# mir-group/allegro

Hardware: AMD Instinct MI355X
Metric: edge tensor-products/sec (forward+force) (higher is better)
Workload: dtype f32; 1 GPU; c4: bulk Si 23^3 cells (97 336 atoms), r_cut 5 A, l_max=2, L=2, u=64; atoms=97336, edges=2725408, parallelism=single GPU, weights=random init (reference initialisers), seed 456, workspace_bytes=21849491824

## Files before the change

### __graft_entry__.py

```python
import os
import sys

ROOT = os.path.dirname(os.path.abspath(__file__))
if ROOT not in sys.path:
    sys.path.insert(0, ROOT)


def build() -> None:
    from allegro_amd.build import build_library, build_torch_ops

    path = build_library(force=True)
    assert os.path.exists(path)
    assert os.path.exists(build_torch_ops(force=True))
    import ctypes

    lib = ctypes.CDLL(path)
    assert lib.aa_version() >= 1
    import allegro_amd
    import allegro_amd.nn
    from oracle import restatement

    print(f"[build] OK: {path}")


def smoke() -> None:
    import torch

    from oracle import restatement as R
    from tests.golden_utils import load_model_fixture
    from tests.hip_utils import fixture_data, model_from_fixture

    assert torch.cuda.is_available(), "smoke() needs a GPU"
    dev = torch.device("cuda:0")
    fx = load_model_fixture("c2", torch.float32)
    model = model_from_fixture(fx, torch.float32, device=dev)
    data, sv = fixture_data(fx, torch.float32, dev)
    g = model.prepare_graph(data["edge_index"], data["atom_types"], data["pos"].shape[0], sv)
    e_atom, forces = model.energy_forces(data["pos"], g)
    torch.cuda.synchronize()
    ref = R.allegro_energy_forces(fx["cfg"], fx["sd"], fx["pos"], fx["edge_index"], fx["types"], fx["shift_vec"])
    de = (e_atom.cpu() - ref["atomic_energy"].reshape(-1)).abs().max().item()
    df = (forces.cpu() - ref["forces"]).abs().max().item()
    dg = (forces.cpu() - fx["out"]["forces"]).abs().max().item()
    print(f"[smoke] C2 fp32 on {torch.cuda.get_device_name(0)}: max|dE_i|={de:.2e} max|dF| vs oracle={df:.2e} "
          f"vs reference golden={dg:.2e} eV/A")
    assert de < 1e-4 and df < 1e-4 and dg < 1e-4, "HIP path disagrees with the oracle"


if __name__ == "__main__":
    build()
    if "--smoke" in sys.argv:
        smoke()
```

### allegro_amd/_lib.py

```python
import ctypes as C
import os
from typing import Optional

import numpy as np

AA_MAX_LAYERS = 4
AA_MAX_MLP_LAYERS = 4
AA_F32, AA_F64 = 0, 1

_dp = C.POINTER(C.c_double)
_ip = C.POINTER(C.c_int32)


class TpDesc(C.Structure):
    _fields_ = [("mul", C.c_int32), ("d1", C.c_int32), ("d2", C.c_int32), ("dout", C.c_int32),
                ("num_paths", C.c_int32), ("coupling", C.c_int32), ("nnz", C.c_int32),
                ("nz_i", _ip), ("nz_j", _ip), ("nz_k", _ip), ("nz_path", _ip), ("nz_val", _dp)]


class ModelConfig(C.Structure):
    _fields_ = [("dtype", C.c_int32), ("num_types", C.c_int32), ("num_bessels", C.c_int32), ("poly_p", C.c_double),
                ("l_max", C.c_int32), ("num_layers", C.c_int32), ("num_scalar", C.c_int32), ("num_tensor", C.c_int32),
                ("embed_dim", C.c_int32), ("embed_mlp_depth", C.c_int32), ("embed_mlp_width", C.c_int32),
                ("latent_mlp_depth", C.c_int32), ("latent_mlp_width", C.c_int32),
                ("readout_mlp_depth", C.c_int32), ("readout_mlp_width", C.c_int32),
                ("forward_weight_init", C.c_int32), ("avg_num_neighbors", C.c_double), ("act_const", C.c_double),
                ("has_scales", C.c_int32), ("has_shifts", C.c_int32), ("tps", TpDesc * AA_MAX_LAYERS),
                ("embed_kind", C.c_int32), ("spline_span", C.c_int32), ("env_shared_weights", C.c_int32),
                ("act_kind", C.c_int32 * 3), ("act_consts", C.c_double * 3), ("bessel_convention", C.c_int32)]


class PlanOptions(C.Structure):
    _fields_ = [(n, C.c_int32) for n in (
        "tp_generic", "tp_no_chain", "tp_no_moments", "tp_no_operator", "tp_force_operator", "tp_operator_fused",
        "gemm_no_chain", "gemm_fp32_mfma", "gemm_valu", "gemm_v1", "gemm_lds_epilogue", "f64_column_loop",
        "embed_no_fuse", "fused_forward", "moments_waves_per_block", "f64_rows", "no_channel_padding", "poison_workspace", "no_slot_form", "op_proj_gemm", "op_env_vector", "staged_no_fold", "op_recompute_bvecs", "readout_two_pass", "tp_prefer_moments", "fused_narrow", "chain_staged_weights")]


def options_from_env() -> PlanOptions:
    env = os.environ
    flag = lambda k: int(env.get(k, "0")[:1] == "1")
    o = PlanOptions()
    o.tp_generic, o.tp_no_chain, o.tp_no_moments = flag("AA_TP_GENERIC"), flag("AA_TP_NOCHAIN"), flag("AA_TP_NOMOM")
    o.tp_no_operator, o.tp_force_operator, o.tp_operator_fused = flag("AA_TP_NOOP"), flag("AA_TP_OP"), flag("AA_OP_NOSPLIT")
    o.gemm_no_chain, o.gemm_fp32_mfma, o.gemm_valu, o.gemm_v1 = (flag("AA_GEMM_NOCHAIN"), flag("AA_GEMM_FP32_MFMA"),
                                                                 flag("AA_GEMM_VALU"), flag("AA_GEMM_V1"))
    o.gemm_lds_epilogue = int(env.get("AA_GEMM_DIRECT_EPILOGUE", "1")[:1] == "0")
    o.f64_column_loop = {"0": 1, "2": 2}.get(env.get("AA_F64_NLOOP", "1")[:1], 0)
    o.embed_no_fuse = flag("AA_EMBED_NOFUSE")
    o.fused_forward = {"0": 3, "1": 1, "2": 2, "4": 4}.get(env.get("AA_FUSED", "")[:1], 0)
    o.moments_waves_per_block = int(env.get("AA_MOM_WPB", "0") or 0)
    o.no_channel_padding = flag("AA_NO_PAD")
    o.no_slot_form = flag("AA_NO_SLOT_FORM")
    o.op_proj_gemm = {"1": 1, "0": 2}.get(env.get("AA_OP_PROJ", "")[:1], 0)
    o.op_env_vector = flag("AA_OP_ENV_VECTOR")
    o.staged_no_fold = flag("AA_STAGED_NOFOLD")
    o.op_recompute_bvecs = flag("AA_OP_RECOMPUTE_BVECS")
    o.readout_two_pass = flag("AA_READOUT_TWO_PASS")
    o.tp_prefer_moments = flag("AA_TP_PREFER_MOM")
    o.fused_narrow = {"1": 1, "2": 2, "3": 3, "4": 4}.get(env.get("AA_FUSED_NARROW", "")[:1], 0)
    o.chain_staged_weights = flag("AA_CHAIN_STAGED")
    o.poison_workspace = flag("AA_POISON")
    o.f64_rows = {"0": 2, "2": 1}.get(env.get("AA_F64_ROWS", "")[:1], 0)
    return o


class RawWeights(C.Structure):
    _fields_ = [("rmax_recip", _dp), ("bessel_weights", _dp), ("center_embed", _dp), ("neighbor_embed", _dp),
                ("basis_linear", _dp), ("embed_mlp", _dp * AA_MAX_MLP_LAYERS), ("env_embed_linear", _dp),
                ("first_proj", _dp), ("latent", (_dp * AA_MAX_MLP_LAYERS) * AA_MAX_LAYERS),
                ("tp_weights", _dp * AA_MAX_LAYERS), ("readout", _dp * AA_MAX_MLP_LAYERS), ("scales", _dp),
                ("shifts", _dp), ("spline_weights", _dp)]


class Graph(C.Structure):
    _fields_ = [("num_atoms", C.c_int64), ("num_edges", C.c_int64), ("center", C.c_void_p), ("nbr", C.c_void_p),
                ("rowptr", C.c_void_p), ("types", C.c_void_p), ("shift_vec", C.c_void_p),
                ("t_rowptr", C.c_void_p), ("t_perm", C.c_void_p), ("atom_begin", C.c_int64), ("atom_end", C.c_int64),
                ("max_degree", C.c_int64)]


class PairZbl(C.Structure):
    _fields_ = [("num_types", C.c_int32), ("atomic_numbers", _dp), ("qqr2e", C.c_double), ("poly_p", C.c_double)]


class GemmSeg(C.Structure):
    _fields_ = [("p", C.c_void_p), ("ld", C.c_int32), ("n", C.c_int32)]


class GemmDesc(C.Structure):
    _fields_ = [("dtype", C.c_int32), ("K", C.c_int32), ("N", C.c_int32), ("M", C.c_int64),
                ("a_count", C.c_int32), ("c_count", C.c_int32), ("a", GemmSeg * 3), ("c", GemmSeg * 3),
                ("c_accum", C.c_int32 * 3), ("has_z", C.c_int32), ("has_add", C.c_int32), ("z", GemmSeg * 3),
                ("add", GemmSeg * 3), ("act_a", C.c_int32), ("act_lo", C.c_int32), ("act_hi", C.c_int32),
                ("act_kind", C.c_int32), ("batch", C.c_int32), ("a_bs", C.c_int64), ("c_bs", C.c_int64),
                ("bsel4", C.c_uint64), ("num_weights", C.c_int32), ("weights", C.c_void_p), ("force_kernel", C.c_int32),
                ("v1", C.c_int32), ("lds_epilogue", C.c_int32), ("f64_rows", C.c_int32), ("f64_column_loop", C.c_int32)]


GEMM_FORMS = {name: i for i, name in enumerate((
    "NONE",
    "F64_VALU", "F64_MFMA", "F64_PIPE_GRID", "F64_PIPE_LOOP", "F64_ROWS_ACC", "F64_ROWS_OPND", "F64_ROWS_ACC_BATCHED",
    "F64_ROWS_OPND_BATCHED", "F64_VALU_EACH", "F64_MFMA_EACH", "F64_PIPE_GRID_EACH", "F64_PIPE_LOOP_EACH",
    "F32_VALU", "F32_MFMA_V1", "F32_V3_K2", "F32_V3_K4", "F32_V3_KS", "F32_BF16X3_K2", "F32_BF16X3_K4", "F32_BF16X3_KS",
    "F32_BF16X3_LDS_K2", "F32_BF16X3_LDS_K4", "F32_BF16X3_LDS_KS", "F32_BF16X3_BATCHED_K2", "F32_BF16X3_BATCHED_K4",
    "F32_BF16X3_BATCHED_KS", "F32_VALU_EACH", "F32_MFMA_V1_EACH", "F32_V3_EACH", "F32_BF16X3_LDS_EACH"))}


class AllegroError(RuntimeError):
    pass


def make_tp_desc(mul, d1, d2, dout, num_paths, coupling, nz_i, nz_j, nz_k, nz_path, nz_val):
    arrs = [np.ascontiguousarray(a, dtype=np.int32) for a in (nz_i, nz_j, nz_k, nz_path)]
    val = np.ascontiguousarray(nz_val, dtype=np.float64)
    d = TpDesc(int(mul), int(d1), int(d2), int(dout), int(num_paths), int(bool(coupling)), int(len(val)),
               arrs[0].ctypes.data_as(_ip), arrs[1].ctypes.data_as(_ip), arrs[2].ctypes.data_as(_ip),
               arrs[3].ctypes.data_as(_ip), val.ctypes.data_as(_dp))
    return d, arrs + [val]


class NlInput(C.Structure):
    _fields_ = [("num_atoms", C.c_int64), ("pos", C.c_void_p), ("cell", C.c_double * 9), ("pbc", C.c_int32 * 3),
                ("dtype", C.c_int32), ("r_cut", C.c_double)]


class NlTypes(C.Structure):
    _fields_ = [("num_types", C.c_int32), ("types_are_int64", C.c_int32), ("cutoffs", _dp), ("atom_types", C.c_void_p)]


class PruneInput(C.Structure):
    _fields_ = [("num_atoms", C.c_int64), ("num_edges", C.c_int64), ("pos", C.c_void_p), ("dtype", C.c_int32),
                ("rowptr", C.c_void_p), ("nbr", C.c_void_p), ("shift_vec", C.c_void_p)]


class EdgeList(C.Structure):
    _fields_ = [("num_atoms", C.c_int64), ("num_edges", C.c_int64), ("edge_index", C.c_void_p), ("row_stride", C.c_int64),
                ("index_is_int64", C.c_int32), ("dtype", C.c_int32), ("pos", C.c_void_p), ("shift_vec", C.c_void_p)]


class Frames(C.Structure):
    _fields_ = [("num_frames", C.c_int32), ("frame_atoms", C.c_void_p)]


# ... 233 lines not shown
```

### allegro_amd/csrc/aa_common.h

```cpp
#pragma once
#include <type_traits>
#include <hip/hip_runtime.h>

#include <algorithm>
#include <cmath>
#include <cstdint>
#include <cstdio>
#include <cstring>
#include <string>
#include <vector>

#include "allegro_amd.h"

extern __shared__ unsigned char aa_smem[];

namespace aa {

void set_error(const std::string& msg);
int fail(int code, const std::string& msg);
int device_cu_count();

#define AA_CHECK_HIP(expr)                                                                      \
  do {                                                                                          \
    hipError_t _e = (expr);                                                                     \
// ... 129 lines not shown
  sn = (q & 1) ? c : s;
  cs = (q & 1) ? s : c;
  if (q & 2) sn = -sn;
  if ((q + 1) & 2) cs = -cs;
}
__device__ __forceinline__ float aa_sin(float x) {
  float s, c;
  aa_sincos(x, s, c);
  return s;
}
__device__ __forceinline__ double aa_sin(double x) { return sin(x); }
__device__ __forceinline__ float aa_cos(float x) {
  float s, c;
  aa_sincos(x, s, c);
  return c;
}
__device__ __forceinline__ double aa_cos(double x) { return cos(x); }
__device__ __forceinline__ float aa_pow(float x, float y) {
  const int n = int(y);
  if (float(n) == y && n >= 0 && n <= 32) {
    float r = 1.f, b = x;
    for (int m = n; m; m >>= 1) {
      if (m & 1) r *= b;
      b *= b;
    }
    return r;
  }
  return powf(x, y);
}
__device__ __forceinline__ double aa_pow(double x, double y) { return pow(x, y); }
__device__ __forceinline__ float aa_sqrt(float x) { return sqrtf(x); }
__device__ __forceinline__ double aa_sqrt(double x) { return sqrt(x); }

__device__ __forceinline__ int sh_l_of(int i) { return i < 1 ? 0 : (i < 4 ? 1 : (i < 9 ? 2 : 3)); }

struct Seg {
  void* p;
  int ld;
  int n;
};
struct SegList {
  int count;
  Seg s[3];
};

struct GemmArgs {
  int64_t M;
  int K, N;
  SegList a;
  const void* B;
  const void* Bp;
  const void* Bq;
  SegList c;
  int c_accum[3];
  int has_z;
  SegList z;
  int act_a;
  int act_lo, act_hi;
  int has_add;
  SegList add;
  int force_kernel;
  int act_kind;
  int opt_v1, opt_lds_epilogue, opt_f64_column_loop, opt_f64_rows;
  int batch;
  int64_t a_bs, c_bs, b_bs, bp_bs, bq_bs;
  unsigned long long bsel4;
};
template <typename T>
int launch_gemm(const GemmArgs& g, hipStream_t stream);

struct ChainLayer {
  GemmArgs g;
  int use_prev;
  int keep_tile;
  int keep_act;
  int a_mode;
  const void* a2_add;
  const void* a2_z;
  int ld_a2add, ld_a2z;
  void* embrev_out;
  void* edge_sum_out;
  void* kept_out;
  int ld_kept;
};
struct ChainArgs {
  int64_t M;
  int nlayers;
  ChainLayer L[4];
  const void* ro_w;
  double ro_factor;
  const void* ro_scales;
  const int32_t* types;
  const int32_t* center;
  const int32_t* nbr;
  const void* emb_table;
  int num_types;
};
int launch_gemm_chain(const ChainArgs& c, hipStream_t stream);
struct ChainB2Args {
  int64_t M;
  const float* a;
  const float* add;
  const float* z;
  int lda, ldadd, ldz;
  const void* Wq;
  float* c0;
  float* c1;
  int ldc0, ldc1;
};
int launch_chain_b2_resident(const ChainB2Args& g, hipStream_t stream);
size_t gemm_packed_elems(int K, int N);
void gemm_pack_b(const double* B, int K, int N, double* out);
size_t gemm_bf16x3_words(int K, int N);
void gemm_pack_bf16x3(const float* B, int K, int N, unsigned* out);

struct TpGroup {
  int32_t out_idx;
  int32_t path;
  int32_t begin, end;
};
struct TpEntry {
  int32_t a, b;
  float val_f;
  double val_d;
};
struct TpTable {
  int32_t num_groups;
  const TpGroup* groups;
  const TpEntry* entries;
};
struct TpLayerDev {
  int32_t mul, d1, d2, dout, num_paths, coupling;
  TpTable fwd;
  TpTable bx1;
  TpTable bx2;
};

struct TpOperand {
  const void* dense;
  const void* sh;
  const void* w;
  int ldw;
  int ld_sh;
};
struct TpOperandGrad {
  void* dense;
  void* gw;
  int ldgw;
  void* gsh;
  int ld_gsh;
};

struct TpLayerFwdArgs {
  int64_t E, N;
  const int32_t* rowptr;
  const int32_t* eids;
  TpOperand x1, x2;
  const void* weights;
  double scatter_factor;
  void* x2s;
  void* out;
  void* scal;
  int ld_scal;
};
struct TpLayerBwdArgs {
  int64_t E, N;
// ... 55 lines not shown
  const void* weights;
  int coupling;
  double sf;
  void* x2s;
  void* out;
  void* scal;
  int ld_scal;
};
struct TpSpecBwdArgs {
  int64_t E, N;
  const int32_t* rowptr;
  int u;
  const void* sh;
  int ld_sh;
  const void* w_x1;
  int ld_w1;
  const void* x1_dense;
  const void* w_env;
  int ld_we;
  const void* weights;
  int coupling;
  double sf;
  const void* x2s;
  const void* gout;
  const void* gscal;
  int ld_gscal;
  void* g_x1_dense;
  void* g_w1;
  int ld_gw1;
  void* g_wenv;
  int ld_gwe;
  void* gsh_x1;
  void* gsh_env;
  int ld_gsh;
};
struct TpChainArgs {
  int64_t E, N;
  int64_t atom0;
  const int32_t* rowptr;
  int u;
  const void* sh;
  int ld_sh;
  const void* w0;
  int ld_w0;
  const void* wenv0;
  int ld_we0;
  const void* wenv1;
  int ld_we1;
  const void* weights0;
  const void* weights1;
  int coupling;
  double sf;
  const void* x2s0;
  void* x2s1;
  void* scal1;
  int ld_scal;
  const void* gscal0;
  const void* gscal1;
  int ld_gscal;
  void* g_w0;
  int ld_gw0;
  void* g_wenv;
  int ld_gwe;
  void* gsh_x1;
  void* gsh_env;
  int ld_gsh;
};
int find_chain_pair(int sig0, int sig1);

struct TpMomArgs {
  TpChainArgs c;
  const void* a0;
  int ld_a0, ka0;
  const void* a1;
  int ld_a1, ka1;
  const void* wk0;
  const void* wt0;
  const void* wk1;
  const void* wt1;
  void* g_a;
  int ld_ga;
  int ka_lds;
  int waves_per_block;
};
struct TpOpArgs {
  int64_t N, E;
  int64_t atom0;
  const int32_t* rowptr;
  int u;
  const void* sh;
  int ld_sh;
  const void* w0;
  int ld_w0;
  int coupling;
  double sf;
  const void* x2s[3];
  const void* tpw[3];
  const void* a;
  int ld_a, ka, act;
  const void* wk;
  const void* wt;
  void* scal;
  int ld_scal;
  const void* gscal[3];
  int ld_gscal;
  void* q;
  void* g_w0;
  int ld_gw0;
  void* gsh_x1;
  void* gsh_env;
  int ld_gsh;
  void* g_a;
  int ld_ga;
  int ka_lds;
  void* bvec;
  void* gmbuf;
  void* mbuf;
  int num_layers;
  int proj_gemm;
  void* dx2s;
  int env_mfma;
  int bvec_ready;
};
int find_op_chain(const int* sigs, int num_layers);
template <typename T>
int launch_tp_op(int chain, int layer, bool reverse, const TpOpArgs& a, hipStream_t stream, int phase = 0);

template <typename T>
int launch_tp_mom_fwd_first(int pair, const TpMomArgs& a, hipStream_t stream);
template <typename T>
int launch_tp_mom_fwd_last(int pair, const TpMomArgs& a, hipStream_t stream);
template <typename T>
int launch_tp_mom_bwd_last(int pair, const TpMomArgs& a, hipStream_t stream);
template <typename T>
int launch_tp_mom_bwd_first(int pair, const TpMomArgs& a, hipStream_t stream);
template <typename T>
int launch_tp_chain_fwd_last(int pair, const TpChainArgs& a, hipStream_t stream);
template <typename T>
int launch_tp_chain_bwd_last(int pair, const TpChainArgs& a, hipStream_t stream);
template <typename T>
int launch_tp_chain_bwd_first(int pair, const TpChainArgs& a, hipStream_t stream);

int find_spec_sig(const aa_tp_desc& d);

struct TpDenseArgs {
  int64_t E, N;
  const int32_t* rowptr;
  const int32_t* eids;
  int u, coupling;
  double sf;
  const void* x1;
  const void* x2;
  const void* weights;
  void* x2s;
  void* out;
  const void* gout;
  void* gx1;
  void* gx2;
};
bool tp_dense_supported(int sig, int u, int dtype);
template <typename T>
int launch_tp_dense(int sig, bool backward, const TpDenseArgs& a, hipStream_t stream);
template <typename T>
int launch_tp_dense_wgrad(int sig, int u, int coupling, const TpLayerWgradArgs& a, hipStream_t stream);
template <typename T>
int launch_tp_spec_fwd(int sig, const TpSpecFwdArgs& a, hipStream_t stream);
template <typename T>
int launch_tp_spec_bwd(int sig, const TpSpecBwdArgs& a, hipStream_t stream);

constexpr int kFusedMaxSteps = 56;
constexpr int kFusedKeepDefault = 2;
constexpr int kFusedMaxDegree = 128;
constexpr int kFusedTailAtomsPerCu = 64;
constexpr int kFusedTeamTilesSmall = 4096;
struct FusedFwdArgs {
  int64_t N, atom0, atom_end;
  int32_t* tile_atoms;
  int32_t* tile_counts;
  int64_t tile_cap;
  const int32_t *rowptr, *nbr, *types;
  const float* pos;
  const float* shift_vec;
  int num_types, embed_kind, spline_span;
  float poly_p;
  const float *rmax_recip, *bessel_w;
  const float* emb_tab;
  const void* wstep[kFusedMaxSteps][2];
  const float *tpw0, *tpw1;
  int coupling;
  float sf;
  const float* ro_w;
  float ro_factor;
  const float *scales, *shifts;
  float* vec;
  float* sh;
  float* se_h;
  float* emb;
  float* w0;
  float* lat_h0;
  float* lat_h1;
  float* ro_h;
  float* fcat;
  float *x2s0, *x2s1;
  float* atom_energy;
  int long_only;
  int32_t* status;
  int mixed;
  int skip_long, fill_done;
  float* g_fcat;
  float* g_scal1;
  int ld_gfcat;
  float* g_scal0;
  float* gsh_env1;
};
size_t fused_fwd_lds_bytes(int num_types, bool teams);
enum class FusedForm { OneWave, FourWave, EightWave, EightWaveTail, EightWaveDeepTail };
int fused_fwd_num_steps(int R);
int launch_fused_fwd(int pair, FusedForm form, const FusedFwdArgs& a, const FusedFwdArgs* wide, hipStream_t stream);
// ... 153 lines not shown
```

### allegro_amd/csrc/aa_gemm.hip

```cpp
#include "aa_common.h"
#include "aa_mfma.h"

namespace aa {


template <typename T>
__device__ __forceinline__ T seg_load(const SegList& sl, int64_t row, int col) {
  int c = col;
#pragma unroll
  for (int s = 0; s < 3; ++s) {
    if (s < sl.count) {
      if (c < sl.s[s].n) return static_cast<const T*>(sl.s[s].p)[row * sl.s[s].ld + c];
      c -= sl.s[s].n;
    }
  }
  return T(0);
}

__device__ __forceinline__ bool a_act(const GemmArgs& g, int k) { return g.act_a && (g.act_hi == 0 || (k >= g.act_lo && k < g.act_hi)); }

template <typename T>
__device__ __forceinline__ void seg_store(const GemmArgs& g, int64_t row, int col, T v) {
  int c = col;
#pragma unroll
// ... 939 lines not shown
#pragma unroll
        for (int q = 0; q < 6; ++q) {
          wn0[q] = p0[q * 64];
          wn1[q] = p1[q * 64];
        }
        __builtin_amdgcn_sched_barrier(0);
        v4f a2[4];
        const int k2 = kc + 2 < KC ? kc + 2 : KC - 1;
        load_a_frag_acc(g, gm, k2, hh, a2, a_sh);
        __builtin_amdgcn_sched_barrier(0);
        u32x4 x1[2], x2[2], x3[2];
        split3_pack(a0, x1, x2, x3);
        chunk_pair_bf16x3(wc0, wc1, x1, x2, x3, acc0, acc1);
#pragma unroll
        for (int q = 0; q < 4; ++q) {
          a0[q] = a1[q];
          a1[q] = a2[q];
        }
#pragma unroll
        for (int q = 0; q < 6; ++q) {
          wc0[q] = wn0[q];
          wc1[q] = wn1[q];
        }
      }
    }
    if (LDS_EPI) {
      store_pair_lds(g, acc0, acc1, two, reinterpret_cast<float*>(aa_smem) + wv * 32 * EP_LD, m0, nt * 32, lane);
    } else {
      store_tile_t(g, acc0, gm, nt * 32, lane, vec_ok, c_sh);
      if (two) store_tile_t(g, acc1, gm, nt * 32 + 32, lane, vec_ok, c_sh);
    }
  }
}


__device__ __forceinline__ void tile_epilogue_store(const GemmArgs& g, v16f& acc, int64_t gm, int n0, int lane) {
#pragma unroll
  for (int gq = 0; gq < 4; ++gq) {
    const int f0 = n0 + 8 * gq + 4 * (lane >> 5);
    const Dst4 d = resolve4(g, gm, f0);
    if (d.nvalid == 0) continue;
    v4f v = {acc[4 * gq], acc[4 * gq + 1], acc[4 * gq + 2], acc[4 * gq + 3]};
    if (d.add) {
      const v4f ad = *reinterpret_cast<const v4f*>(d.add);
#pragma unroll
      for (int e = 0; e < 4; ++e) v[e] += ad[e];
    }
    if (d.z) {
      const v4f z = *reinterpret_cast<const v4f*>(d.z);
#pragma unroll
      for (int e = 0; e < 4; ++e) v[e] *= dsilu(z[e]);
    }
#pragma unroll
    for (int e = 0; e < 4; ++e) acc[4 * gq + e] = v[e];
    if (d.c) {
      if (d.accum) {
        const v4f o = *reinterpret_cast<const v4f*>(d.c);
#pragma unroll
        for (int e = 0; e < 4; ++e) v[e] += o[e];
      }
      *reinterpret_cast<v4f*>(d.c) = v;
    }
  }
}

constexpr int kChainMaxBlocks = 12;
struct ChainTileDev {
  float* c;
  const float* z;
  const float* add;
  int ldc, ldz, ldadd, accum;
};
struct ChainLayerDev {
  const u32x4* Wq;
  int KCg, KC, NT;
  int keep_tile, keep_act, a_mode, pad_;
  int use_prev, pad2_;
  float* edge_sum_out;
  float* embrev_out;
  float* kept_out;
  int ld_kept, pad3_;
  const float *a2_add, *a2_z;
  int ld_a2add, ld_a2z;
  const float* a[kChainMaxBlocks];
  int lda[kChainMaxBlocks];
  ChainTileDev t[kChainMaxBlocks];
};
struct ChainDev {
  int64_t M;
  int nlayers;
  float ro_factor;
  const float* ro_w;
  const float* ro_scales;
  const int32_t* types;
  const int32_t* center;
  int ro_n;
  const int32_t* nbr;
  const float* emb_table;
  int num_types;
  ChainLayerDev L[4];
};

constexpr int kEpLd = 36;

template <bool PRE, bool EMB>
__global__ __launch_bounds__(256, PRE ? 2 : 3) void gemm_chain_bf16x3_kernel(ChainDev c) {
  auto chain_split = [](const v4f* a, u32x4* l1, u32x4* l2, u32x4* l3) {
    if constexpr (PRE)
      split3_pack_masked(a, l1, l2, l3);
    else
      split3_pack(a, l1, l2, l3);
  };
  u32x4* wbuf = reinterpret_cast<u32x4*>(aa_smem);
  const int tid = threadIdx.x, lane = tid & 63, wv = tid >> 6;
  const int64_t m0 = (int64_t(blockIdx.x) * 4 + wv) * 32;
  const int64_t gm = m0 + (lane & 31);
  const int hh = lane >> 5;
  const bool row_ok = gm < c.M;
  const int64_t gmc = row_ok ? gm : c.M - 1;
  v16f kept0, kept1;
#pragma unroll
  for (int r = 0; r < 16; ++r) {
    kept0[r] = 0.f;
    kept1[r] = 0.f;
  }
  float rofac = c.ro_factor;
  if (c.ro_scales) rofac *= c.ro_scales[c.types[c.center[gmc]]];
  float* sRo = reinterpret_cast<float*>(wbuf + 2 * kWStep);
  for (int i = tid; i < c.ro_n; i += 256) sRo[i] = c.ro_w[i];
  float* sT = sRo + 32 * kChainMaxBlocks + wv * 32 * kEpLd;
  const float* sTab = sRo + 32 * kChainMaxBlocks + 4 * 32 * kEpLd;
  if (EMB && c.emb_table) {
    float* tab = const_cast<float*>(sTab);
    for (int i = tid; i < c.num_types * c.num_types * 512; i += 256) tab[i] = c.emb_table[i];
    sTab += (c.types[c.center[gmc]] * c.num_types + c.types[c.nbr[gmc]]) * 512;
  }
  auto stage_load = [&](const ChainLayerDev& L, int nt, int kc, u32x4* r) {
    const size_t chunk_stride = 64 * 6, tile_stride = size_t(L.KC) * chunk_stride;
    const int t1 = nt + 1 < L.NT ? nt + 1 : nt;
    const u32x4* s0 = L.Wq + size_t(nt) * tile_stride + size_t(kc) * chunk_stride;
    const u32x4* s1 = L.Wq + size_t(t1) * tile_stride + size_t(kc) * chunk_stride;
    r[0] = s0[tid];
    r[1] = tid < 128 ? s0[256 + tid] : s1[tid - 128];
    r[2] = s1[128 + tid];
  };
  auto stage_write = [&](int b, const u32x4* r) {
    u32x4* d = wbuf + b * kWStep;
    d[tid] = r[0];
    d[256 + tid] = r[1];
    d[512 + tid] = r[2];
  };
  auto load_a = [&](const ChainLayerDev& L, int kc, v4f* a) {
    const float* p = L.a[kc] + gmc * L.lda[kc] + 4 * hh;
#pragma unroll
    for (int q = 0; q < 4; ++q) a[q] = *reinterpret_cast<const v4f*>(p + 8 * q);
  };
  auto finish_a = [&](const ChainLayerDev& L, int kc, v4f* a) {
    if (L.a_mode == 1) {
      const float* rw = sRo + kc * 32 + 4 * hh;
#pragma unroll
      for (int q = 0; q < 4; ++q) {
        const v4f wv4 = *reinterpret_cast<const v4f*>(rw + 8 * q);
#pragma unroll
        for (int e = 0; e < 4; ++e) a[q][e] = rofac * wv4[e] * dsilu(a[q][e]);
      }
    }
  };
  auto finish_a2 = [&](const ChainLayerDev& L, int kc, v4f* a) {
    const float* pa = L.a2_add + gmc * L.ld_a2add + kc * 32 + 4 * hh;
    const float* pz = L.a2_z + gmc * L.ld_a2z + kc * 32 + 4 * hh;
    v4f ad[4], zz[4];
#pragma unroll
    for (int q = 0; q < 4; ++q) {
      ad[q] = *reinterpret_cast<const v4f*>(pa + 8 * q);
      zz[q] = *reinterpret_cast<const v4f*>(pz + 8 * q);
    }
#pragma unroll
    for (int q = 0; q < 4; ++q)
#pragma unroll
      for (int e = 0; e < 4; ++e) a[q][e] = (a[q][e] + ad[q][e]) * dsilu(zz[q][e]);
  };
  auto kept_a = [&](const ChainLayerDev& L, int j, v4f* a) {
    const bool first = (j & 1) == 0;
#pragma unroll
    for (int q = 0; q < 4; ++q)
#pragma unroll
      for (int e = 0; e < 4; ++e) a[q][e] = first ? kept0[4 * q + e] : kept1[4 * q + e];
  };
  auto mma_step = [&](int b, const u32x4* x1, const u32x4* x2, const u32x4* x3, v16f& acc0, v16f& acc1) {
    const u32x4* w = wbuf + b * kWStep + lane;
#define AA_W(T_, Q_) w[((T_)*6 + (Q_)) * 64]
    {
      const u32x4 a0 = AA_W(0, 4), b0 = AA_W(1, 4), a1 = AA_W(0, 5), b1 = AA_W(1, 5);
      acc0 = mma_bf16(a0, x1[0], acc0);
      acc1 = mma_bf16(b0, x1[0], acc1);
      acc0 = mma_bf16(a1, x1[1], acc0);
      acc1 = mma_bf16(b1, x1[1], acc1);
    }
    {
      const u32x4 a0 = AA_W(0, 2), b0 = AA_W(1, 2), a1 = AA_W(0, 3), b1 = AA_W(1, 3);
      acc0 = mma_bf16(a0, x2[0], acc0);
      acc1 = mma_bf16(b0, x2[0], acc1);
      acc0 = mma_bf16(a1, x2[1], acc0);
      acc1 = mma_bf16(b1, x2[1], acc1);
      acc0 = mma_bf16(a0, x1[0], acc0);
      acc1 = mma_bf16(b0, x1[0], acc1);
      acc0 = mma_bf16(a1, x1[1], acc0);
      acc1 = mma_bf16(b1, x1[1], acc1);
    }
    {
      const u32x4 a0 = AA_W(0, 0), b0 = AA_W(1, 0), a1 = AA_W(0, 1), b1 = AA_W(1, 1);
      acc0 = mma_bf16(a0, x3[0], acc0);
      acc1 = mma_bf16(b0, x3[0], acc1);
      acc0 = mma_bf16(a1, x3[1], acc0);
      acc1 = mma_bf16(b1, x3[1], acc1);
      acc0 = mma_bf16(a0, x2[0], acc0);
      acc1 = mma_bf16(b0, x2[0], acc1);
      acc0 = mma_bf16(a1, x2[1], acc0);
      acc1 = mma_bf16(b1, x2[1], acc1);
      acc0 = mma_bf16(a0, x1[0], acc0);
      acc1 = mma_bf16(b0, x1[0], acc1);
      acc0 = mma_bf16(a1, x1[1], acc0);
      acc1 = mma_bf16(b1, x1[1], acc1);
    }
#undef AA_W
  };
  auto epilogue = [&](const ChainTileDev& d, v16f& acc) {
    const bool has_add = d.add != nullptr, has_z = d.z != nullptr, has_old = d.c != nullptr && d.accum;
    {
      v4f ad[4], zz[4];
      if (has_add) {
        const float* p = d.add + gmc * d.ldadd + 4 * hh;
#pragma unroll
        for (int q = 0; q < 4; ++q) ad[q] = *reinterpret_cast<const v4f*>(p + 8 * q);
      }
      if (has_z) {
        const float* p = d.z + gmc * d.ldz + 4 * hh;
#pragma unroll
        for (int q = 0; q < 4; ++q) zz[q] = *reinterpret_cast<const v4f*>(p + 8 * q);
      }
      if (has_add) {
#pragma unroll
        for (int r = 0; r < 16; ++r) acc[r] += ad[r >> 2][r & 3];
      }
      if (has_z) {
#pragma unroll
        for (int r = 0; r < 16; ++r) acc[r] *= dsilu(zz[r >> 2][r & 3]);
      }
    }
    if (d.c != nullptr) {
      float* st = sT + (lane & 31) * kEpLd + 4 * hh;
#pragma unroll
      for (int q = 0; q < 4; ++q) *reinterpret_cast<v4f*>(st + 8 * q) = v4f{acc[4 * q], acc[4 * q + 1], acc[4 * q + 2], acc[4 * q + 3]};
      __builtin_amdgcn_wave_barrier();
      const int pr = lane >> 3, pc = 4 * (lane & 7);
      v4f v[4];
#pragma unroll
      for (int q = 0; q < 4; ++q) v[q] = *reinterpret_cast<const v4f*>(sT + (8 * q + pr) * kEpLd + pc);
      __builtin_amdgcn_wave_barrier();
      float* p = d.c + (m0 + pr) * d.ldc + pc;
      if (has_old) {
        v4f old[4];
#pragma unroll
        for (int q = 0; q < 4; ++q) {
          const int64_t rr = m0 + pr + 8 * q < c.M ? m0 + pr + 8 * q : c.M - 1;
          old[q] = *reinterpret_cast<const v4f*>(d.c + rr * d.ldc + pc);
        }
#pragma unroll
        for (int q = 0; q < 4; ++q)
#pragma unroll
          for (int e = 0; e < 4; ++e) v[q][e] += old[q][e];
      }
#pragma unroll
      for (int q = 0; q < 4; ++q)
        if (m0 + pr + 8 * q < c.M) *reinterpret_cast<v4f*>(p + int64_t(8 * q) * d.ldc) = v[q];
    }
  };

  const float* const dummy_a = c.L[0].a[0];
  const int dummy_lda = c.L[0].lda[0];
  auto load_rows = [&](const float* base, int ld, v4f* a) {
    const float* p = base + gmc * ld + 4 * hh;
#pragma unroll
    for (int q = 0; q < 4; ++q) a[q] = *reinterpret_cast<const v4f*>(p + 8 * q);
  };
  auto streams = [&](const ChainLayerDev& X) { return X.KCg > 0 && !(PRE && X.KC <= 2 && X.NT > 2); };
  int step = 0;
  {
    u32x4 r[3];
    stage_load(c.L[0], 0, 0, r);
    stage_write(0, r);
  }
  v4f a0[4];
  load_rows(dummy_a, dummy_lda, a0);
  __syncthreads();
  for (int li = 0; li < c.nlayers; ++li) {
    const ChainLayerDev& L = c.L[li];
    const int KCg = L.KCg, KC = L.KC, NT = L.NT;
    const bool last_layer = li + 1 >= c.nlayers;
    const ChainLayerDev& Ln = c.L[last_layer ? li : li + 1];
    const bool next_streams = !last_layer && streams(Ln);
    const bool pre = PRE && KC <= 2 && NT > 2;
    u32x4 ps1[PRE ? 2 : 1][2], ps2[PRE ? 2 : 1][2], ps3[PRE ? 2 : 1][2];
    if constexpr (PRE) {
      if (pre) {
#pragma unroll
        for (int kc = 0; kc < 2; ++kc) {
          if (kc < KC) {
            v4f a[4];
            if (kc >= KCg) {
              kept_a(L, kc - KCg, a);
            } else {
              load_a(L, kc, a);
              if (L.a_mode == 2)
                finish_a2(L, kc, a);
              else
                finish_a(L, kc, a);
            }
            chain_split(a, ps1[kc], ps2[kc], ps3[kc]);
          }
        }
      }
    }
    for (int nt = 0; nt < NT; nt += 2) {
      const bool two = nt + 1 < NT;
      const bool last_pair = nt + 2 >= NT;
      v16f acc0, acc1;
#pragma unroll
      for (int r = 0; r < 16; ++r) {
        acc0[r] = 0.f;
        acc1[r] = 0.f;
      }
      for (int kc = 0; kc < KC; ++kc) {
        const bool lastc = kc + 1 >= KC;
        const bool layer_end = lastc && last_pair;
        const bool kernel_end = layer_end && last_layer;
        u32x4 r[3];
        stage_load(layer_end && !kernel_end ? Ln : L, (layer_end && !kernel_end) ? 0 : (lastc && !kernel_end ? nt + 2 : nt),
                   (lastc && !kernel_end) ? 0 : (kernel_end ? kc : kc + 1), r);
        u32x4 x1[2], x2[2], x3[2];
        if (!pre) {
          if (kc >= KCg) {
            v4f a[4];
            kept_a(L, kc - KCg, a);
            chain_split(a, x1, x2, x3);
          } else {
            finish_a(L, kc, a0);
            chain_split(a0, x1, x2, x3);
          }
        }
        {
          const float* tp = dummy_a;
          int tl = dummy_lda;
          if (!pre && !lastc && kc + 1 < KCg) {
            tp = L.a[kc + 1];
            tl = L.lda[kc + 1];
          } else if (lastc && !last_pair && KCg > 0 && !pre) {
            tp = L.a[0];
            tl = L.lda[0];
          } else if (layer_end && next_streams) {
            tp = Ln.a[0];
            tl = Ln.lda[0];
          }
          load_rows(tp, tl, a0);
        }
        if constexpr (PRE) {
          if (pre) {
            if (kc == 0)
              mma_step(step & 1, ps1[0], ps2[0], ps3[0], acc0, acc1);
            else
              mma_step(step & 1, ps1[1], ps2[1], ps3[1], acc0, acc1);
          } else {
            mma_step(step & 1, x1, x2, x3, acc0, acc1);
          }
        } else {
          mma_step(step & 1, x1, x2, x3, acc0, acc1);
        }
        stage_write((step + 1) & 1, r);
#ifdef AA_CHAIN_SYNCTHREADS
        __syncthreads();
#else
        lds_barrier();
#endif
        ++step;
      }
      epilogue(L.t[nt], acc0);
      if (two) epilogue(L.t[nt + 1], acc1);
      if (EMB && L.embrev_out) {
        float part[8];
#pragma unroll
        for (int n = 0; n < 8; ++n) {
          float p = 0.f;
#pragma unroll
          for (int q = 0; q < 4; ++q) {
            const v4f t0 = *reinterpret_cast<const v4f*>(sTab + n * 64 + 8 * q + 4 * hh);
            const v4f t1 = *reinterpret_cast<const v4f*>(sTab + n * 64 + 32 + 8 * q + 4 * hh);
#pragma unroll
            for (int e = 0; e < 4; ++e) p += acc0[4 * q + e] * t0[e] + acc1[4 * q + e] * t1[e];
          }
          part[n] = p;
        }
        float other[8];
#pragma unroll
        for (int n = 0; n < 8; ++n) other[n] = part[n];
        permlane32_swap4(part, other);
        permlane32_swap4(part + 4, other + 4);
        if (row_ok) {
          const int o4 = 4 * hh;
          *reinterpret_cast<v4f*>(L.embrev_out + gm * 8 + o4) =
              v4f{part[o4] + other[o4], part[o4 + 1] + other[o4 + 1], part[o4 + 2] + other[o4 + 2], part[o4 + 3] + other[o4 + 3]};
        }
      }
      if (L.edge_sum_out) {
        float part = 0.f;
#pragma unroll
        for (int q = 0; q < 4; ++q) {
          const v4f w0v = *reinterpret_cast<const v4f*>(sRo + 8 * q + 4 * hh);
          const v4f w1v = *reinterpret_cast<const v4f*>(sRo + 32 + 8 * q + 4 * hh);
#pragma unroll
          for (int e = 0; e < 4; ++e) part += silu(acc0[4 * q + e]) * w0v[e] + silu(acc1[4 * q + e]) * w1v[e];
        }
        float t = part, o = part;
        permlane32_swap(t, o);
        if (row_ok && hh == 0) L.edge_sum_out[gm] = t + o;
      }
      if (nt == L.keep_tile) {
#pragma unroll
        for (int r = 0; r < 16; ++r) {
          kept0[r] = L.keep_act ? silu(acc0[r]) : acc0[r];
          kept1[r] = L.keep_act ? silu(acc1[r]) : acc1[r];
        }
        if (L.kept_out && row_ok) {
          float* ko = L.kept_out + gm * L.ld_kept + 4 * hh;
#pragma unroll
          for (int q = 0; q < 4; ++q) {
            *reinterpret_cast<v4f*>(ko + 8 * q) = v4f{kept0[4 * q], kept0[4 * q + 1], kept0[4 * q + 2], kept0[4 * q + 3]};
            *reinterpret_cast<v4f*>(ko + 32 + 8 * q) = v4f{kept1[4 * q], kept1[4 * q + 1], kept1[4 * q + 2], kept1[4 * q + 3]};
          }
        }
      }
    }
  }
}

int launch_gemm_chain(const ChainArgs& c, hipStream_t stream) {
  if (c.M == 0) return AA_OK;
  ChainDev d{};
  d.M = c.M;
  d.nlayers = c.nlayers;
  d.ro_factor = float(c.ro_factor);
  d.ro_w = static_cast<const float*>(c.ro_w);
  d.ro_scales = static_cast<const float*>(c.ro_scales);
  d.types = c.types;
  d.center = c.center;
  d.nbr = c.nbr;
  d.emb_table = static_cast<const float*>(c.emb_table);
  d.num_types = c.num_types;
  if (c.emb_table && (c.num_types < 1 || c.num_types > 2 || !c.types || !c.center || !c.nbr))
    return fail(AA_ERR_INVALID, "gemm chain: the embedding table needs 1..2 types and the edge / type arrays");
  if (c.nlayers < 1 || c.nlayers > 4) return fail(AA_ERR_INVALID, "gemm chain: 1..4 layers");
  bool have_kept = false;
  static_assert(sizeof(ChainDev) <= 4096, "kernel argument block too large");
  for (int li = 0; li < c.nlayers; ++li) {
    const ChainLayer& L = c.L[li];
    const GemmArgs& g = L.g;
    ChainLayerDev& D = d.L[li];
    int ka = 0, nc = 0, nchunk = 0, ntile = 0;
    if (g.act_a) return fail(AA_ERR_INVALID, "gemm chain: act_a is not supported");
    for (int s = 0; s < g.a.count; ++s) {
      const Seg& sg = g.a.s[s];
      if ((sg.n & 31) || (sg.ld & 3) || (reinterpret_cast<uintptr_t>(sg.p) & 15) || !sg.p)
        return fail(AA_ERR_INVALID, "gemm chain: A segments must be 32-column granular and 16-B aligned");
      for (int k = 0; k < sg.n; k += 32) {
        if (nchunk >= kChainMaxBlocks) return fail(AA_ERR_INVALID, "gemm chain: too many k chunks");
        D.a[nchunk] = static_cast<const float*>(sg.p) + k;
        D.lda[nchunk] = sg.ld;
        ++nchunk;
      }
      ka += sg.n;
    }
    if (g.has_z && g.z.count != g.c.count) return fail(AA_ERR_INVALID, "gemm chain: z must be split like c");
    if (g.has_add && g.add.count != g.c.count) return fail(AA_ERR_INVALID, "gemm chain: add must be split like c");
    for (int s = 0; s < g.c.count; ++s) {
      const Seg& sg = g.c.s[s];
      if ((sg.n & 31) || (sg.ld & 3) || (reinterpret_cast<uintptr_t>(sg.p) & 15))
        return fail(AA_ERR_INVALID, "gemm chain: C segments must be 32-column granular and 16-B aligned");
      if (g.has_z && (g.z.s[s].n != sg.n || (g.z.s[s].ld & 3) || (reinterpret_cast<uintptr_t>(g.z.s[s].p) & 15) || !g.z.s[s].p))
        return fail(AA_ERR_INVALID, "gemm chain: bad z segment");
      if (g.has_add && (g.add.s[s].n != sg.n || (g.add.s[s].ld & 3) || (reinterpret_cast<uintptr_t>(g.add.s[s].p) & 15) || !g.add.s[s].p))
        return fail(AA_ERR_INVALID, "gemm chain: bad add segment");
      for (int k = 0; k < sg.n; k += 32) {
        if (ntile >= kChainMaxBlocks) return fail(AA_ERR_INVALID, "gemm chain: too many output tiles");
        ChainTileDev& t = D.t[ntile];
        t.c = sg.p ? static_cast<float*>(sg.p) + k : nullptr;
        t.ldc = sg.ld;
        t.accum = g.c_accum[s];
        t.z = g.has_z ? static_cast<const float*>(g.z.s[s].p) + k : nullptr;
        t.ldz = g.has_z ? g.z.s[s].ld : 0;
        t.add = g.has_add ? static_cast<const float*>(g.add.s[s].p) + k : nullptr;
        t.ldadd = g.has_add ? g.add.s[s].ld : 0;
        ++ntile;
      }
      nc += sg.n;
    }
    if (ka + (L.use_prev ? 64 : 0) != g.K || nc != g.N || !g.Bq) return fail(AA_ERR_INVALID, "gemm chain: bad layer shape");
    if (L.keep_tile >= 0 && ((L.keep_tile & 1) || L.keep_tile * 32 + 64 > g.N || (L.use_prev && L.keep_tile * 32 + 64 != g.N)))
      return fail(AA_ERR_INVALID, "gemm chain: the kept 64 features must be a tile pair (the last one of a layer that chains)");
    if (L.use_prev && !have_kept) return fail(AA_ERR_INVALID, "gemm chain: nothing to chain from");
    have_kept = have_kept || L.keep_tile >= 0;
    D.Wq = static_cast<const u32x4*>(g.Bq);
    D.KCg = nchunk;
    D.KC = nchunk + (L.use_prev ? 2 : 0);
    D.use_prev = L.use_prev;
    D.NT = ntile;
    D.keep_tile = L.keep_tile;
    D.keep_act = L.keep_act;
    D.a_mode = L.a_mode;
    if (L.a_mode == 2) {
      if (!L.a2_add || !L.a2_z || (L.ld_a2add & 3) || (L.ld_a2z & 3) || L.use_prev || g.a.count != 1 || !(nchunk <= 2 && ntile > 2))
        return fail(AA_ERR_INVALID, "gemm chain: a_mode 2 needs one A segment of <= 2 chunks, > 2 output tiles, and its add / z arrays");
      D.a2_add = static_cast<const float*>(L.a2_add);
      D.a2_z = static_cast<const float*>(L.a2_z);
      D.ld_a2add = L.ld_a2add;
      D.ld_a2z = L.ld_a2z;
    }
    if (L.a_mode == 1) {
      if (!c.ro_w) return fail(AA_ERR_INVALID, "gemm chain: a_mode 1 needs ro_w");
      d.ro_n = std::max(d.ro_n, nchunk * 32);
    }
    D.kept_out = static_cast<float*>(L.kept_out);
    D.ld_kept = L.ld_kept;
    if (L.kept_out && (L.keep_tile < 0 || (L.ld_kept & 3) || (reinterpret_cast<uintptr_t>(L.kept_out) & 15)))
      return fail(AA_ERR_INVALID, "gemm chain: kept_out needs a kept tile pair and 16-B aligned rows");
    D.embrev_out = static_cast<float*>(L.embrev_out);
    if (L.embrev_out && (!c.emb_table || g.N != 64)) return fail(AA_ERR_INVALID, "gemm chain: embrev_out needs the table and a 64-wide layer");
    D.edge_sum_out = static_cast<float*>(L.edge_sum_out);
    if (L.edge_sum_out) {
      if (!c.ro_w || g.N != 64) return fail(AA_ERR_INVALID, "gemm chain: edge_sum_out needs ro_w and a 64-wide layer");
      d.ro_n = std::max(d.ro_n, 64);
    }
  }
  dim3 grid((unsigned)((c.M + 127) / 128));
  bool any_pre = false;
  for (int li = 0; li < d.nlayers; ++li) any_pre = any_pre || (d.L[li].KC <= 2 && d.L[li].NT > 2);
  const size_t smem = sizeof(u32x4) * 2 * kWStep + sizeof(float) * (32 * kChainMaxBlocks + 4 * 32 * kEpLd) +
                      (c.emb_table ? sizeof(float) * 512 * c.num_types * c.num_types : 0);
  bool emb = false;
  for (int li = 0; li < d.nlayers; ++li) emb = emb || d.L[li].embrev_out != nullptr;
#define AA_CHAIN_LAUNCH(P_, E_) hipLaunchKernelGGL((gemm_chain_bf16x3_kernel<P_, E_>), grid, dim3(256), smem, stream, d)
  if (any_pre) {
    if (emb) AA_CHAIN_LAUNCH(true, true); else AA_CHAIN_LAUNCH(true, false);
  } else {
    if (emb) AA_CHAIN_LAUNCH(false, true); else AA_CHAIN_LAUNCH(false, false);
  }
#undef AA_CHAIN_LAUNCH
  AA_CHECK_HIP(hipGetLastError());
  return AA_OK;
}

size_t gemm_bf16x3_words(int K, int N) { return size_t((N + 31) / 32) * size_t((K + 31) / 32) * 64 * 24; }
void gemm_pack_bf16x3(const float* B, int K, int N, unsigned* out) {
  const int NT = (N + 31) / 32, KC = (K + 31) / 32;
  auto trunc = [](float x) {
    unsigned u;
    memcpy(&u, &x, 4);
    return u & 0xFFFF0000u;
  };
  auto tof = [](unsigned u) {
    float x;
    memcpy(&x, &u, 4);
    return x;
  };
  for (int nt = 0; nt < NT; ++nt)
    for (int kc = 0; kc < KC; ++kc)
      for (int lane = 0; lane < 64; ++lane) {
        unsigned* o = out + (size_t(nt) * KC + kc) * 64 * 24 + size_t(lane) * 4;
        for (int half = 0; half < 2; ++half)
          for (int q = 0; q < 4; ++q) {
            unsigned h[3][2];
            for (int e = 0; e < 2; ++e) {
              int s = half * 8 + q * 2 + e;
              int k = kc * 32 + 8 * (s >> 2) + 4 * (lane >> 5) + (s & 3), n = nt * 32 + (lane & 31);
              float x = (k < K && n < N) ? B[size_t(k) * N + n] : 0.f;
              h[0][e] = trunc(x);
              float r = x - tof(h[0][e]);
              h[1][e] = trunc(r);
              float r2 = r - tof(h[1][e]);
              h[2][e] = trunc(r2);
            }
            for (int lv = 0; lv < 3; ++lv) o[size_t(lv * 2 + half) * 64 * 4 + q] = (h[lv][0] >> 16) | h[lv][1];
          }
      }
}

size_t gemm_packed_elems(int K, int N) { return size_t((N + 31) / 32) * size_t((K + 31) / 32) * 64 * 16; }

void gemm_pack_b(const double* B, int K, int N, double* out) {
  const int NT = (N + 31) / 32, KC = (K + 31) / 32;
  for (int nt = 0; nt < NT; ++nt)
    for (int kc = 0; kc < KC; ++kc)
      for (int lane = 0; lane < 64; ++lane)
        for (int s = 0; s < 16; ++s) {
          int k = kc * 32 + (lane >> 5) * 16 + s, n = nt * 32 + (lane & 31);
          out[((size_t(nt) * KC + kc) * 64 + lane) * 16 + s] = (k < K && n < N) ? B[size_t(k) * N + n] : 0.0;
        }
}

static bool seglist_frag_ok_host(const SegList& sl) {
  for (int s = 0; s < sl.count; ++s)
    if ((sl.s[s].n & 15) || (sl.s[s].ld & 3) || (reinterpret_cast<uintptr_t>(sl.s[s].p) & 15)) return false;
  return true;
}

static int check_args(const GemmArgs& g) {
  int ka = 0, nc = 0;
  for (int s = 0; s < g.a.count; ++s) ka += g.a.s[s].n;
  for (int s = 0; s < g.c.count; ++s) nc += g.c.s[s].n;
  if (ka != g.K || nc != g.N) return fail(AA_ERR_INVALID, "gemm: segment widths do not sum to K/N");
  if (g.batch > 1 && (g.batch > 16 || g.has_z || g.has_add)) return fail(AA_ERR_INVALID, "gemm: batched launches take up to 16 problems and no z / add operands");
  if (g.act_a && g.act_hi != 0 && ((g.act_lo & 31) || (g.act_hi & 31) || g.act_lo < 0 || g.act_hi <= g.act_lo || g.act_hi > g.K))
    return fail(AA_ERR_INVALID, "gemm: the activated column range of A must be 32-granular and inside [0, K)");
  if (g.has_add) {
    if (g.add.count != g.c.count) return fail(AA_ERR_INVALID, "gemm: add/c segment mismatch");
    for (int s = 0; s < g.c.count; ++s)
      if (g.add.s[s].n != g.c.s[s].n) return fail(AA_ERR_INVALID, "gemm: add/c segment mismatch");
  }
  if (g.has_z) {
    if (g.z.count != g.c.count) return fail(AA_ERR_INVALID, "gemm: z/c segment mismatch");
    for (int s = 0; s < g.c.count; ++s)
      if (g.z.s[s].n != g.c.s[s].n) return fail(AA_ERR_INVALID, "gemm: z/c segment mismatch");
  }
  return AA_OK;
}
// ... 373 lines not shown
```

### allegro_amd/csrc/aa_model.hip

```cpp
#include <algorithm>
#include <atomic>

#include "aa_common.h"

namespace aa {
static thread_local std::string g_err;
void set_error(const std::string& msg) { g_err = msg; }
int fail(int code, const std::string& msg) {
  g_err = msg;
  return code;
}
int device_cu_count() {
  constexpr int kMaxDevices = 64;
  static std::atomic<int> cached[kMaxDevices];
  int dev = 0, n = 0;
  AA_CHECK_HIP(hipGetDevice(&dev));
  const bool slot = dev >= 0 && dev < kMaxDevices;
  if (slot && (n = cached[dev].load(std::memory_order_relaxed)) > 0) return n;
  AA_CHECK_HIP(hipDeviceGetAttribute(&n, hipDeviceAttributeMultiprocessorCount, dev));
  if (n <= 0) return fail(AA_ERR_HIP, "hipDeviceGetAttribute: the device reports no compute units");
  if (slot) cached[dev].store(n, std::memory_order_relaxed);
  return n;
}
}
// ... 230 lines not shown
    if (pad) d.mul = u;
    m.spec_sig[l] = find_spec_sig(d);
    sigs_ok = sigs_ok && m.spec_sig[l] >= 0;
  }
  const bool spec = sigs_ok && !(q.dtype == AA_F64 && q.l_max >= 3);
  const int chain_pair = (spec && L == 2 && !opt.tp_no_chain) ? find_chain_pair(m.spec_sig[0], m.spec_sig[1]) : -1;
  const bool moments_ok = scalars_ok && latents_ok && chain_pair >= 0 && u == 64 &&
                          (f32 ? 4 : 8) * 4 * Dsh * (std::max(S, H) + 64 + 64) <= 160 * 1024;
  const bool operator_ok = scalars_ok && latents_ok && sigs_ok && L >= 2 && L <= 3 && (u % 64) == 0 && u <= 256 && !opt.tp_no_operator;
  const bool prefer_op = moments_ok && !chains_shape && (slot_shape || !f32) && !opt.tp_prefer_moments;
  const int tp_op = (operator_ok && (!moments_ok || opt.tp_force_operator || prefer_op)) ? find_op_chain(m.spec_sig, L) : -1;
  m.tp = tp_op >= 0 ? TpPath::Operator : moments_ok ? TpPath::Moments : chain_pair >= 0 ? TpPath::SpecChain : spec ? TpPath::Spec : TpPath::General;
  m.chain_pair = chain_pair;
  m.tp_op = tp_op;
  m.op_proj = tp_op >= 0 && opt.op_proj_gemm != 2;

  const bool chains = m.env_moments() && (tp_op < 0 || u == 64) && chains_shape;
  m.linear = chains ? LinearPath::Chains : (tp_op >= 0 && slot_shape) ? LinearPath::Slot : LinearPath::Single;
  const bool tab_ok = chains && T <= 3 && B == 8 && S0 == 64;
  m.two_body_table = tab_ok || q.embed_kind == 1;
  m.embed_fused = tab_ok && T <= 2 && !opt.embed_no_fuse;
  m.fold_embed_table = tab_ok;
  const bool chains2 = chains && L == 2;
  m.fold_embed_output = chains2;
  m.fold_latent_outputs = chains2;
  m.fold_lat0_reverse = chains2;

  const bool fused = m.tp == TpPath::Moments && (chain_pair == 0 || chain_pair == 1) && m.fold_embed_table && m.fold_embed_output &&
                     m.fold_latent_outputs && opt.fused_forward != 3;
  m.fused_fwd = fused;
  m.fused_wide = fused && opt.fused_narrow != 1 && fused_fwd8_lds_bytes(T, 8) <= 160 * 1024;
  m.num_tensor = u;
  m.embed_width = He;
  m.latent_width = H;
  m.readout_width = Hr;
  return m;
}

struct StepInputs {
  bool f32;
  bool taps;
  bool with_forces;
  bool transposed_csr;
  int64_t atoms, edges;
  int64_t atom0, atom_end;
  int64_t max_degree;
  bool pair_zbl;
  bool block;
};

enum class ForwardKind {
  Staged,
  StagedFolded,
  FusedOneTile,
  FusedTeam,
  FusedMixed,
};
enum class ReverseInForward {
  None = 0,
  Chain = 1,
  ChainMomentsLatent0 = 2,
};
enum class LatentReverse {
  Mlp,
  TwoLayerChain,
  FoldedChain,
  Resident,
  InForwardTail,
};

struct StepPlan {
  ForwardKind forward;
  FusedForm fused_form;
  bool slot;
  bool op_split;
  bool op_split_reverse;
  bool proj_forward, proj_reverse;
  bool readout_grad_in_reduce;
  ReverseInForward reverse_in_forward;
  LatentReverse latent_reverse;
  bool gather;
  bool zero_gsh, zero_forces;
  bool pair_zbl;
  bool block;

  bool fused() const { return forward == ForwardKind::FusedOneTile || forward == ForwardKind::FusedTeam || forward == ForwardKind::FusedMixed; }
  bool folded_first_stage() const { return forward != ForwardKind::Staged; }
};

static ReverseInForward fused_tail(FusedForm form) {
  return form == FusedForm::EightWaveDeepTail ? ReverseInForward::ChainMomentsLatent0
         : form == FusedForm::EightWaveTail   ? ReverseInForward::Chain
                                              : ReverseInForward::None;
}

static ForwardKind choose_forward(const ModelPipeline& pipe, const aa_plan_options& opt, const aa_model_config& c, const StepInputs& in) {
  const bool fold_staged = pipe.chains() && pipe.tp_op < 0 && pipe.fold_embed_output && pipe.fold_latent_outputs && c.num_layers == 2 && !in.taps &&
                           !opt.staged_no_fold;
  const ForwardKind staged = fold_staged ? ForwardKind::StagedFolded : ForwardKind::Staged;
  if (!(in.f32 && pipe.fused_fwd && !in.taps && in.max_degree > 0 && in.max_degree <= kFusedMaxDegree)) return staged;
  const bool long_segments = in.max_degree > 32;
  if (fused_fwd_lds_bytes(c.num_types, long_segments) > size_t(160) * 1024) return staged;
  if (!long_segments) return ForwardKind::FusedOneTile;
  const int64_t n_active = in.atom_end - in.atom0;
  const int64_t tiles = n_active * (in.max_degree <= 64 ? 2 : 4);
  const double fill = double(in.edges) / (32.0 * double(std::max<int64_t>(n_active, 1)));
  const bool avg_fits_one_tile = fill <= 1.15;
  const ForwardKind team = opt.fused_forward == 2 ? ForwardKind::FusedTeam
                           : (opt.fused_forward == 4 || avg_fits_one_tile) ? ForwardKind::FusedMixed
                                                                           : ForwardKind::FusedTeam;
  if (opt.fused_forward == 2 || opt.fused_forward == 4) return team;
  if (fill >= 0.6 && avg_fits_one_tile) return team;
  return (tiles <= kFusedTeamTilesSmall || double(in.edges) >= 0.85 * 32.0 * double(tiles)) ? team : staged;
}

static bool wide_one_tile_pass(const ModelPipeline& pipe, ForwardKind forward) {
  return pipe.fused_wide && (forward == ForwardKind::FusedOneTile || forward == ForwardKind::FusedMixed);
}

static StepPlan choose_step(const ModelPipeline& pipe, const aa_plan_options& opt, const aa_model_config& c, const StepInputs& in, int cus) {
  const int64_t n = in.atom_end - in.atom0;
  const bool two_layer_chains = pipe.chains() && c.num_layers == 2;
  StepPlan s{};
  s.forward = choose_forward(pipe, opt, c, in);

  const bool resident_shape = in.f32 && c.num_scalar == 64 && c.num_tensor == 64;
  const bool tail_ok = in.with_forces && s.forward == ForwardKind::FusedOneTile && two_layer_chains && pipe.fold_latent_outputs;
  const bool deep_ok = tail_ok && pipe.fold_lat0_reverse && pipe.env_moments() && resident_shape && c.latent_mlp_width == 64 && opt.fused_narrow != 4;
  const FusedForm tail_form = deep_ok ? FusedForm::EightWaveDeepTail : FusedForm::EightWaveTail;
  s.fused_form = !wide_one_tile_pass(pipe, s.forward)                ? FusedForm::OneWave
                 : (opt.fused_narrow == 2 || opt.fused_narrow == 4) ? (tail_ok ? tail_form : FusedForm::EightWave)
                 : opt.fused_narrow == 3                             ? FusedForm::FourWave
                 : n <= int64_t(4) * cus                             ? FusedForm::OneWave
                 : (tail_ok && n >= int64_t(kFusedTailAtomsPerCu) * cus) ? tail_form
                                                                         : FusedForm::FourWave;
  s.reverse_in_forward = n > 0 ? fused_tail(s.fused_form) : ReverseInForward::None;

  s.slot = pipe.slot() && !in.taps;
  s.readout_grad_in_reduce = in.with_forces && !pipe.chains() && c.readout_mlp_depth > 0 && !opt.readout_two_pass;
  s.latent_reverse = !pipe.chains()                                                     ? LatentReverse::Mlp
                     : s.reverse_in_forward == ReverseInForward::ChainMomentsLatent0 ? LatentReverse::InForwardTail
                     : !(pipe.fold_lat0_reverse && c.num_layers == 2)                ? LatentReverse::TwoLayerChain
                     : (resident_shape && !opt.chain_staged_weights)                 ? LatentReverse::Resident
                                                                                     : LatentReverse::FoldedChain;

  s.op_split = pipe.tp_op >= 0 && !opt.tp_operator_fused;
  s.op_split_reverse = s.op_split && in.with_forces;
  s.proj_forward = pipe.op_proj && s.op_split && (opt.op_proj_gemm == 1 || n >= 4096);
  s.proj_reverse = s.proj_forward && in.with_forces;

  s.block = in.block;
  s.gather = in.transposed_csr || (s.block && in.with_forces);
  s.zero_gsh = in.with_forces && !((pipe.channel_minor() && c.num_tensor <= 64) || pipe.tp_op >= 0);
  s.zero_forces = in.with_forces && !s.gather;
  s.pair_zbl = in.pair_zbl;
  return s;
}

struct MlpLayout {
  std::vector<int> dims;
  std::vector<size_t> w, wt;
  std::vector<size_t> wp, wtp;
  std::vector<size_t> wq, wtq;
};

struct GemmMat {
  size_t w = 0, wp = 0, wq = 0;
  int K = 0, N = 0;
};

struct GemmMatSet {
  size_t w = 0, wp = 0, wq = 0, w_bs = 0, wp_bs = 0, wq_bs = 0;
  int K = 0, N = 0, count = 0;
};

static std::vector<int> mlp_dims(int in, int depth, int width, int out) {
  std::vector<int> d{in};
  for (int i = 0; i < depth; ++i) d.push_back(width);
  d.push_back(out);
  return d;
}

struct BlobLayout {
  size_t o_rmax = 0, o_bessel = 0, o_cemb = 0, o_nemb = 0, o_basis = 0, o_g0 = 0, o_g0t = 0, o_g0p = 0, o_g0tp = 0, o_g0q = 0, o_g0tq = 0,
         o_b3a_q = 0, o_b3b_q = 0, o_b3c_q = 0, o_ro_last = 0, o_scales = 0, o_shifts = 0, n_elems = 0;
  size_t o_tpw[AA_MAX_LAYERS] = {};
  MlpLayout embed, readout;
  MlpLayout latent[AA_MAX_LAYERS];
  int ro_last_dim = 0;
  size_t o_embtab = 0;
  size_t o_embtab_h = 0;
  size_t o_lat1in_fq = 0, o_ro0_fq = 0;
  size_t o_b3af_q = 0;
  size_t o_b3bf_q = 0;
  size_t o_g0fq = 0, o_g0tfq = 0;
  size_t o_wk0f = 0, o_wt0f = 0;
  GemmMat s_g0f, s_g0ft;
  GemmMat s_in[AA_MAX_LAYERS];
  GemmMat s_ro0;
  GemmMat s_rs[AA_MAX_LAYERS];
  GemmMat s_rstb;
  GemmMat s_sct[AA_MAX_LAYERS];
  size_t o_s_wk0 = 0, o_s_wt0 = 0;
  GemmMatSet s_pr[AA_MAX_LAYERS], s_prt[AA_MAX_LAYERS], s_pr0f, s_prt0f;
  int ng0 = 0;
  size_t o_wk[AA_MAX_LAYERS] = {}, o_wt[AA_MAX_LAYERS] = {};

  uint64_t hash(const aa_model_config& c, const ModelPipeline& pipe, int u_raw) const;
};

static BlobLayout layout_blob(const aa_model_config& c, const ModelPipeline& pipe) {
  BlobLayout b;
  const int L = c.num_layers, S = c.num_scalar, u = c.num_tensor, T = c.num_types, B = c.num_bessels, S0 = c.embed_dim;
  const int R = c.l_max + 1, W = R * u, SL1 = S * (L + 1), Hr = c.readout_mlp_width, H = c.latent_mlp_width;
  size_t o = 0;
  auto take = [&](size_t n) {
    size_t r = o;
    o += (n + 63) / 64 * 64;
    return r;
  };
  auto lay = [&](MlpLayout& m, const std::vector<int>& dims, int nlayers) {
    m.dims = dims;
    for (int i = 0; i < nlayers; ++i) {
      m.w.push_back(take(size_t(dims[i]) * dims[i + 1]));
      m.wt.push_back(take(size_t(dims[i]) * dims[i + 1]));
      m.wp.push_back(take(gemm_packed_elems(dims[i], dims[i + 1])));
      m.wtp.push_back(take(gemm_packed_elems(dims[i + 1], dims[i])));
// ... 773 lines not shown
}

extern "C" int aa_model_pack_weights(const aa_model_plan* p, const aa_model_raw_weights* raw, void* dev_blob, size_t blob_bytes,
                                     aa_stream stream) {
  AA_REQUIRE(p && raw && dev_blob, "aa_model_pack_weights: null argument");
  AA_REQUIRE(blob_bytes >= aa_model_weights_bytes(p), "aa_model_pack_weights: blob too small");
  std::vector<unsigned char> bytes;
  if (int rc = pack_blob_host(*p, *raw, bytes)) return rc;
  hipStream_t s = static_cast<hipStream_t>(stream);
  AA_CHECK_HIP(hipMemcpyAsync(dev_blob, bytes.data(), bytes.size(), hipMemcpyHostToDevice, s));
  AA_CHECK_HIP(hipStreamSynchronize(s));
  return AA_OK;
}

struct Workspace {
  size_t vec, sh, emb0, emb, w0, fcat, g_fcat, g_envw, g_w0, g_emb, g_emb0, g_sh, g_ro_last, g_aenv, e_edge, q_op, bvec_op, gm_op, mom_op, dx2s_op, trev, dvec, vir_part, tiles;
  size_t g_scal[AA_MAX_LAYERS];
  size_t se_h[AA_MAX_MLP_LAYERS], g_se_h[AA_MAX_MLP_LAYERS];
  size_t envw[AA_MAX_LAYERS], x2s[AA_MAX_LAYERS], tf[AA_MAX_LAYERS], scal[AA_MAX_LAYERS];
  size_t lat_h[AA_MAX_LAYERS][AA_MAX_MLP_LAYERS], g_lat_h[AA_MAX_MLP_LAYERS];
  size_t ro_h[AA_MAX_MLP_LAYERS], g_ro_h[AA_MAX_MLP_LAYERS];
  size_t g_tf[2];
  size_t total;
};

static int num_gsh_slots(const aa_model_plan* p) {
  const aa_model_config& c = p->cfg;
  if (p->pipe.tp_op >= 0) {
    int n = c.num_tensor / 64;
    for (int l = 0; l < c.num_layers; ++l) n += (l == 0 ? c.num_scalar : c.latent_mlp_width) / 64;
    return n;
  }
  return p->pipe.channel_minor() ? c.num_layers + 1 : 1;
}

static Workspace layout_workspace(const aa_model_plan* p, int64_t N, int64_t E, int with_forces) {
  Workspace w{};
  const aa_model_config& c = p->cfg;
  const size_t es = p->esize();
  size_t o = 0;
  auto take = [&](size_t elems) {
    size_t r = o;
    o += (elems * es + 255) / 256 * 256;
    return r;
  };
  const int S = c.num_scalar, u = c.num_tensor, L = c.num_layers, S0 = c.embed_dim;
  const size_t Ez = size_t(E), Nz = size_t(N);
  w.vec = take(Ez * 4);
  w.sh = take(Ez * p->D);
  w.emb0 = take(Ez * S0);
  for (int i = 0; i < c.embed_mlp_depth; ++i) w.se_h[i] = take(Ez * c.embed_mlp_width);
  w.emb = take(Ez * S);
  w.w0 = take(Ez * p->W);
  w.fcat = take(Ez * p->SL1);
  size_t dmax = 1;
  for (int l = 0; l < L; ++l) {
    if (!p->pipe.env_moments()) w.envw[l] = take(Ez * p->W);
    w.x2s[l] = take(Nz * u * p->D);
    if (l < L - 1 && p->pipe.chain_pair < 0 && !p->pipe.env_moments()) {
      w.tf[l] = take(Ez * u * c.tps[l].dout);
      dmax = std::max(dmax, size_t(c.tps[l].dout));
    }
    w.scal[l] = take(Ez * u);
    for (int i = 0; i < c.latent_mlp_depth; ++i) w.lat_h[l][i] = take(Ez * c.latent_mlp_width);
  }
  for (int i = 0; i < c.readout_mlp_depth; ++i) w.ro_h[i] = take(Ez * c.readout_mlp_width);
  if (p->pipe.chains()) w.e_edge = take(Ez);
  if (p->pipe.embed_fused) w.trev = take(Ez * 8);
  if (p->pipe.fused_fwd) w.tiles = take(((3 * Nz + 8) * sizeof(int32_t) + es - 1) / es);
  if (with_forces) {
    w.dvec = take(Ez * 4);
    w.vir_part = take((size_t(kVirialBlocks) * 9 * sizeof(double) + es - 1) / es);
  }
  if (p->pipe.tp_op >= 0) {
    w.bvec_op = take(Nz * L * p->D * u);
    w.mom_op = take(Nz * p->D * size_t(std::max(c.num_scalar, c.latent_mlp_width)));
  }
  if (with_forces) {
    w.g_fcat = take(Ez * p->SL1);
    for (int i = 0; i < c.readout_mlp_depth; ++i) w.g_ro_h[i] = take(Ez * c.readout_mlp_width);
    for (int i = 0; i < c.latent_mlp_depth; ++i) w.g_lat_h[i] = take(Ez * c.latent_mlp_width);
    for (int l = 0; l < L; ++l) w.g_scal[l] = take(Ez * u);
    if (!p->pipe.env_moments()) w.g_envw = take(Ez * p->W);
    if (p->pipe.env_moments()) w.g_aenv = take(Ez * size_t(std::max(S, c.latent_mlp_width)));
    w.g_w0 = take(Ez * p->W);
    if (L > 1 && p->pipe.chain_pair < 0) {
      w.g_tf[0] = take(Ez * u * dmax);
      w.g_tf[1] = L > 2 ? take(Ez * u * dmax) : w.g_tf[0];
    }
    w.g_emb = take(Ez * S);
    for (int i = 0; i < c.embed_mlp_depth; ++i) w.g_se_h[i] = take(Ez * c.embed_mlp_width);
    w.g_emb0 = take(Ez * S0);
    w.g_sh = take(Ez * p->D * num_gsh_slots(p));
    if (p->pipe.tp_op >= 0) {
      w.q_op = take(Nz * L * p->D * u);
      w.gm_op = take(Nz * p->D * size_t(std::max(c.num_scalar, c.latent_mlp_width)));
      if (p->pipe.op_proj) w.dx2s_op = take(Nz * p->D * u);
    }
  }
  w.total = o;
  return w;
}

extern "C" size_t aa_model_workspace_bytes(const aa_model_plan* plan, int64_t N, int64_t E, int with_forces) {
  if (!plan) return 0;
  return layout_workspace(plan, N, E, with_forces).total;
}

struct BlockedWorkspace {
  Workspace arena;
  size_t rowptr, bad, vec, dvec, total;
};
static BlockedWorkspace layout_blocked(const aa_model_plan* p, int64_t N, int64_t E, int64_t max_block_edges, int with_forces) {
  BlockedWorkspace b{};
  b.arena = layout_workspace(p, N, max_block_edges, with_forces);
  size_t o = b.arena.total;
  auto take = [&](size_t bytes) {
    size_t r = o;
    o += (bytes + 255) / 256 * 256;
    return r;
  };
  b.rowptr = take(sizeof(int32_t) * (size_t(N) + 1));
  b.bad = take(sizeof(int32_t));
  if (with_forces) {
    b.vec = take(size_t(E) * 4 * p->esize());
    b.dvec = take(size_t(E) * 4 * p->esize());
  }
  b.total = o;
  return b;
}

extern "C" size_t aa_model_blocked_workspace_bytes(const aa_model_plan* plan, int64_t N, int64_t E, int64_t max_block_edges, int with_forces) {
  if (!plan || N < 0 || E < 0 || max_block_edges < 0) return 0;
  return layout_blocked(plan, N, E, std::min(max_block_edges, E), with_forces).total;
}

namespace {

inline Seg seg(void* p, int ld, int n) { return Seg{p, ld, n}; }

struct StageProfile {
  std::vector<std::string> names;
  std::vector<hipEvent_t> events;
  std::vector<double> bytes, flops;
  int mark(const char* name, hipStream_t s, double by, double fl) {
    hipEvent_t e;
    AA_CHECK_HIP(hipEventCreate(&e));
    AA_CHECK_HIP(hipEventRecord(e, s));
    names.emplace_back(name);
    events.push_back(e);
    bytes.push_back(by);
    flops.push_back(fl);
    return AA_OK;
  }
  void clear() {
    for (hipEvent_t e : events) (void)hipEventDestroy(e);
    events.clear();
    names.clear();
    bytes.clear();
    flops.clear();
  }
};

template <typename T>
struct Runner {
  const aa_model_plan* p;
  const T* wts;
// ... 150 lines not shown
    r.center = g->center;
    r.types = g->types;
    if (c.readout_mlp_depth > 0) {
      r.h = buf(w.ro_h[c.readout_mlp_depth - 1]);
      r.ld = c.readout_mlp_width;
      r.H = c.readout_mlp_width;
      r.act = 1;
    } else {
      r.h = buf(w.fcat);
      r.ld = p->SL1;
      r.H = p->SL1;
      r.act = 0;
    }
    r.w = wt(p->blob.o_ro_last);
    r.act_kind = c.act_kind[2];
    r.factor = 1.0 / std::sqrt(2.0 * c.avg_num_neighbors);
    r.scales = c.has_scales ? wt(p->blob.o_scales) : nullptr;
    r.shifts = c.has_shifts ? wt(p->blob.o_shifts) : nullptr;
    r.atom_energy = atom_energy;
    r.edge_sum = (p->pipe.chains() && atom_energy) ? buf(w.e_edge) : nullptr;
    return r;
  }

  int64_t atom_begin(const aa_graph* g) const { return g->atom_end > g->atom_begin ? g->atom_begin : 0; }
  int64_t atom_end(const aa_graph* g) const { return g->atom_end > g->atom_begin ? g->atom_end : N; }

  TpChainArgs chain_args(const aa_graph* g) const {
    const aa_model_config& c = p->cfg;
    TpChainArgs a{};
    a.E = E;
    a.N = N;
    a.rowptr = g->rowptr;
    a.u = c.num_tensor;
    a.sh = buf(w.sh);
    a.ld_sh = p->D;
    a.w0 = buf(w.w0);
    a.ld_w0 = p->W;
    a.wenv0 = buf(w.envw[0]);
    a.ld_we0 = p->W;
    a.wenv1 = buf(w.envw[1]);
    a.ld_we1 = p->W;
    a.weights0 = wt(p->blob.o_tpw[0]);
    a.weights1 = wt(p->blob.o_tpw[1]);
    a.coupling = c.tps[0].coupling;
    a.sf = 1.0 / std::sqrt(c.avg_num_neighbors);
    a.x2s0 = buf(w.x2s[0]);
    a.x2s1 = buf(w.x2s[1]);
    a.scal1 = buf(w.scal[1]);
    a.ld_scal = c.num_tensor;
    a.ld_gscal = c.num_tensor;
    a.ld_gw0 = p->W;
    a.ld_gwe = p->W;
    a.ld_gsh = p->D;
    return a;
  }

  static ChainLayer chain_layer(int64_t M, const SegList& a, int act_a, const void* Bq, int K, int Nn, const SegList& c,
                                const int* accum, const SegList* z, const SegList* add, int use_prev, int keep_tile,
                                int keep_act) {
    ChainLayer L{};
    L.g.M = M;
    L.g.K = K;
    L.g.N = Nn;
    L.g.a = a;
    L.g.Bq = Bq;
    L.g.c = c;
    for (int i = 0; i < 3; ++i) L.g.c_accum[i] = accum ? accum[i] : 0;
    L.g.has_z = z ? 1 : 0;
    if (z) L.g.z = *z;
    L.g.has_add = add ? 1 : 0;
    if (add) L.g.add = *add;
    L.g.act_a = act_a;
    L.use_prev = use_prev;
    L.keep_tile = keep_tile;
    L.keep_act = keep_act;
    return L;
  }
  int run_chain(ChainArgs& ca, const char* tag) {
    ca.M = E;
    if (int rc = launch_gemm_chain(ca, stream)) return rc;
    if (!prof) return AA_OK;
    char nm[32];
    int o = snprintf(nm, sizeof(nm), "gc");
    double elems = 0, fl = 0;
    for (int i = 0; i < ca.nlayers; ++i) {
      if (o < 28) o += snprintf(nm + o, sizeof(nm) - o, "_%dx%d", ca.L[i].g.K, ca.L[i].g.N);
      elems += gemm_row_elems(ca.L[i].g, true);
      if (ca.L[i].a_mode == 2) elems += 2.0 * ca.L[i].g.a.s[0].n;
      fl += 2.0 * double(E) * ca.L[i].g.K * ca.L[i].g.N;
    }
    (void)tag;
    return mark(nm, elems, 0, fl);
  }

  TpMomArgs mom_args(const aa_graph* g) const {
    const aa_model_config& c = p->cfg;
    TpMomArgs m{};
    m.c = chain_args(g);
    m.c.atom0 = atom_begin(g);
    m.c.N = atom_end(g);
    m.c.wenv0 = m.c.wenv1 = nullptr;
    m.a0 = buf(w.emb);
    m.ld_a0 = c.num_scalar;
    m.ka0 = c.num_scalar;
    m.a1 = buf(w.lat_h[0][c.latent_mlp_depth - 1]);
    m.ld_a1 = c.latent_mlp_width;
    m.ka1 = c.latent_mlp_width;
    m.wk0 = wt(p->blob.o_wk[0]);
    m.wt0 = wt(p->blob.o_wt[0]);
    m.wk1 = wt(p->blob.o_wk[1]);
    m.wt1 = wt(p->blob.o_wt[1]);
    m.waves_per_block = p->opt.moments_waves_per_block;
    return m;
  }

  TpOpArgs op_args(const aa_graph* g, int l) const {
    const aa_model_config& c = p->cfg;
    TpOpArgs o{};
    o.N = atom_end(g);
    o.atom0 = atom_begin(g);
    o.E = E;
    o.rowptr = g->rowptr;
    o.u = c.num_tensor;
    o.sh = buf(w.sh);
    o.ld_sh = p->D;
    o.w0 = buf(w.w0);
    o.ld_w0 = p->W;
    o.coupling = c.tps[0].coupling;
    o.sf = 1.0 / std::sqrt(c.avg_num_neighbors);
    for (int m = 0; m < c.num_layers && m < 3; ++m) {
      o.x2s[m] = buf(w.x2s[m]);
      o.tpw[m] = wt(p->blob.o_tpw[m]);
    }
    if (l == 0) {
      o.a = buf(w.emb);
      o.ld_a = o.ka = c.num_scalar;
      o.act = 0;
    } else {
      o.a = buf(w.lat_h[l - 1][c.latent_mlp_depth - 1]);
      o.ld_a = o.ka = c.latent_mlp_width;
      o.act = 1;
    }
    o.wk = wt(p->blob.o_wk[l]);
    o.wt = wt(p->blob.o_wt[l]);
    if (sp.slot) {
      if (l == 0) {
        o.a = buf(w.se_h[c.embed_mlp_depth - 1]);
        o.ld_a = o.ka = c.embed_mlp_width;
        o.act = 1;
        o.wk = wt(p->blob.o_s_wk0);
        o.wt = wt(p->blob.o_s_wt0);
      } else {
        o.a = buf(w.fcat) + size_t(c.num_scalar) * l;
        o.ld_a = p->SL1;
      }
    }
    o.ld_scal = c.num_tensor;
    o.ld_gscal = c.num_tensor;
    o.q = buf(w.q_op);
    o.num_layers = c.num_layers;
    o.bvec = sp.op_split ? buf(w.bvec_op) : nullptr;
    o.gmbuf = sp.op_split_reverse ? buf(w.gm_op) : nullptr;
    o.mbuf = sp.op_split ? buf(w.mom_op) : nullptr;
    o.ld_gw0 = p->W;
    o.ld_gsh = p->D;
    o.ka_lds = std::max(c.num_scalar, c.latent_mlp_width);
    o.env_mfma = (sizeof(T) == 8 && !p->opt.op_env_vector && (o.ld_a % 2) == 0) ? 1 : 0;
    return o;
  }

  int proj_gemm(const TpOpArgs& o, const GemmMatSet& ms, const T* a_base, int64_t a_ld, int64_t a_bs, T* c_base, int64_t c_ld, int64_t c_bs) {
    GemmArgs gm{};
    gm.M = o.N - o.atom0;
    gm.K = ms.K;
    gm.N = ms.N;
// ... 606 lines not shown
  int bwd_latent(int l) {
    const aa_model_config& c = p->cfg;
    const int S = c.num_scalar, u = c.num_tensor, L = c.num_layers, W = p->W, SL1 = p->SL1;
    if (p->pipe.chains() && l == L - 1) return AA_OK;
    const SegList none{0, {}};
    ChainArgs ca{};
    SegList in{1, {seg(buf(w.g_fcat) + S * (l + 1), SL1, S)}};
    SegList c1{2, {seg(buf(w.g_fcat), SL1, S * (l + 1)), seg(buf(w.g_scal[l]), u, u)}};
    int acc1[3] = {1, 0, 0};
    switch (sp.latent_reverse) {
      case LatentReverse::Mlp: {
        SegList go;
        go.count = (l < L - 1 && !p->pipe.env_moments()) ? 2 : 1;
        go.s[0] = seg(buf(w.g_fcat) + S * (l + 1), SL1, S);
        if (l < L - 1 && !p->pipe.env_moments()) go.s[1] = seg(buf(w.g_envw), W, W);
        SegList aenv{1, {seg(p->pipe.env_moments() ? buf(w.g_aenv) : nullptr, c.latent_mlp_width, c.latent_mlp_width)}};
        const SegList* addp = (p->pipe.env_moments() && l < L - 1) ? &aenv : nullptr;
        return mlp_bwd(p->blob.latent[l], c.latent_mlp_depth + 1, go, w.lat_h[l], w.g_lat_h, c1, acc1, 1, addp);
      }
      case LatentReverse::InForwardTail:
        return AA_OK;
      case LatentReverse::TwoLayerChain: {
        ca.nlayers = 2;
        SegList cn{1, {seg(nullptr, 64, 64)}};
        SegList zz{1, {seg(buf(w.lat_h[l][0]), 64, 64)}};
        SegList ad{1, {seg(buf(w.g_aenv), 64, 64)}};
        ca.L[0] = chain_layer(E, in, 0, wt(p->blob.latent[l].wtq[1]), S, 64, cn, nullptr, &zz, &ad, 0, 0, 0);
        ca.L[1] = chain_layer(E, none, 0, wt(p->blob.latent[l].wtq[0]), 64, S * (l + 1) + u, c1, acc1, nullptr, nullptr, 1, -1, 0);
        return run_chain(ca, "B2");
      }
      case LatentReverse::FoldedChain:
      case LatentReverse::Resident:
        ca.nlayers = 1;
        ca.L[0] = chain_layer(E, in, 0, wt(p->blob.latent[l].wtq[0]), 64, S * (l + 1) + u, c1, acc1, nullptr, nullptr, 0, -1, 0);
        ca.L[0].a_mode = 2;
        ca.L[0].a2_add = buf(w.g_aenv);
        ca.L[0].ld_a2add = 64;
        ca.L[0].a2_z = buf(w.lat_h[l][0]);
        ca.L[0].ld_a2z = 64;
        if (sp.latent_reverse == LatentReverse::FoldedChain) return run_chain(ca, "B2");
        {
          ChainB2Args b2{};
          b2.M = E;
          b2.a = reinterpret_cast<const float*>(buf(w.g_fcat)) + S * (l + 1);
          b2.lda = SL1;
          b2.add = reinterpret_cast<const float*>(buf(w.g_aenv));
          b2.ldadd = 64;
          b2.z = reinterpret_cast<const float*>(buf(w.lat_h[l][0]));
          b2.ldz = 64;
          b2.Wq = wt(p->blob.latent[l].wtq[0]);
          b2.c0 = reinterpret_cast<float*>(buf(w.g_fcat));
          b2.ldc0 = SL1;
          b2.c1 = reinterpret_cast<float*>(buf(w.g_scal[l]));
          b2.ldc1 = u;
          if (int rc = launch_chain_b2_resident(b2, stream)) return rc;
          return mark("gc_64x128", gemm_row_elems(ca.L[0].g, true) + 2.0 * 64, 0, 2.0 * double(E) * 64 * 128);
        }
    }
    return fail(AA_ERR_INVALID, "step plan: unknown latent reverse form");
  }

  int bwd_tp_layer(const aa_graph* g, int l) {
    const aa_model_config& c = p->cfg;
    const int S = c.num_scalar, u = c.num_tensor, L = c.num_layers, W = p->W;
    switch (p->pipe.tp) {
      case TpPath::Operator:
        return run_op_bwd(g, l);
      case TpPath::Moments: {
        if (l == 1 && sp.reverse_in_forward == ReverseInForward::ChainMomentsLatent0) return AA_OK;
        TpMomArgs m = mom_args(g);
        m.c.gscal0 = buf(w.g_scal[0]);
        m.c.gscal1 = buf(w.g_scal[1]);
        m.c.g_w0 = buf(w.g_w0);
        m.c.gsh_x1 = buf(w.g_sh);
        m.c.gsh_env = buf(w.g_sh) + size_t(l + 1) * size_t(E) * p->D;
        m.g_a = buf(w.g_aenv);
        if (l == 1) {
          m.ld_ga = c.latent_mlp_width;
          if (int rc = launch_tp_mom_bwd_last<T>(p->pipe.chain_pair, m, stream)) return rc;
          return mark("tp_mom_bwd_last", p->D + W + u + 2 * m.ka1 + p->D, double(p->D) * u);
        }
        m.ld_ga = S;
        if (sp.folded_first_stage()) m.wt0 = wt(p->blob.o_wt0f);
        if (int rc = launch_tp_mom_bwd_first<T>(p->pipe.chain_pair, m, stream)) return rc;
        return mark("tp_mom_bwd_first", p->D + 2 * W + 2 * u + 2 * m.ka0 + 2 * p->D, 2.0 * p->D * u);
      }
      case TpPath::SpecChain: {
        TpChainArgs a = chain_args(g);
        a.gscal0 = buf(w.g_scal[0]);
        a.gscal1 = buf(w.g_scal[1]);
        a.g_w0 = buf(w.g_w0);
        a.g_wenv = buf(w.g_envw);
        a.gsh_x1 = buf(w.g_sh);
        a.gsh_env = buf(w.g_sh) + size_t(l + 1) * size_t(E) * p->D;
        if (l == 1) {
          if (int rc = launch_tp_chain_bwd_last<T>(p->pipe.chain_pair, a, stream)) return rc;
          return mark("tp_chain_bwd_last", 3 * W + 2 * p->D + u, 2.0 * p->D * u);
        }
        if (int rc = launch_tp_chain_bwd_first<T>(p->pipe.chain_pair, a, stream)) return rc;
        return mark("tp_chain_bwd_first", 4 * W + 3 * p->D + 2 * u, 2.0 * p->D * u);
      }
      case TpPath::Spec: {
        TpSpecBwdArgs a{};
        spec_operands(a, g, l);
        if (l == 0) {
          a.g_w1 = buf(w.g_w0);
          a.ld_gw1 = W;
        } else {
          a.g_x1_dense = buf(w.g_tf[(l - 1) & 1]);
        }
        a.gout = l < L - 1 ? buf(w.g_tf[l & 1]) : nullptr;
        a.gscal = buf(w.g_scal[l]);
        a.ld_gscal = u;
        a.g_wenv = buf(w.g_envw);
        a.ld_gwe = W;
        a.gsh_x1 = buf(w.g_sh);
        a.gsh_env = buf(w.g_sh) + size_t(l + 1) * size_t(E) * p->D;
        a.ld_gsh = p->D;
        if (int rc = launch_tp_spec_bwd<T>(p->pipe.spec_sig[l], a, stream)) return rc;
        return mark("tp_spec_bwd", 4 * W + 3 * p->D + 2 * u * p->D + u, 2.0 * p->D * u);
      }
      case TpPath::General: {
        TpLayerBwdArgs a{};
        general_operands(a, g, l);
        a.gout = l < L - 1 ? buf(w.g_tf[l & 1]) : nullptr;
        a.gscal = buf(w.g_scal[l]);
        a.ld_gscal = u;
        if (l == 0) {
          a.g1.gw = buf(w.g_w0);
          a.g1.ldgw = W;
          a.g1.gsh = buf(w.g_sh);
          a.g1.ld_gsh = p->D;
        } else {
          a.g1.dense = buf(w.g_tf[(l - 1) & 1]);
        }
        a.g2.gw = buf(w.g_envw);
        a.g2.ldgw = W;
        a.g2.gsh = buf(w.g_sh);
        a.g2.ld_gsh = p->D;
        if (int rc = launch_tp_layer_bwd<T>(p->layers[l], a, stream)) return rc;
        return mark("tp_layer_bwd", 4 * W + 2 * p->D + 2 * u * p->D + u, 2.0 * p->D * u);
      }
    }
    return fail(AA_ERR_INVALID, "step plan: unknown tensor-product path");
  }

  int bwd_first_stage(const aa_graph* g) {
    const aa_model_config& c = p->cfg;
    const int S = c.num_scalar, W = p->W, SL1 = p->SL1;
    if (!p->pipe.chains()) {
      {
        SegList go{3, {seg(buf(w.g_fcat), SL1, S), seg(buf(w.g_w0), W, W), seg(buf(w.g_envw), W, W)}};
        if (p->pipe.env_moments()) go.count = 2;
        SegList gi{1, {seg(buf(w.g_emb), S, S)}};
        SegList aenv{1, {seg(p->pipe.env_moments() ? buf(w.g_aenv) : nullptr, S, S)}};
        act_now = AA_ACT_SILU;
        if (int rc = gemm(go, 0, wt(p->blob.o_g0t), wt(p->blob.o_g0tp), wt(p->blob.o_g0tq), p->blob.ng0, S, gi, nullptr, nullptr,
                          p->pipe.env_moments() ? &aenv : nullptr))
          return rc;
      }
      SegList go{1, {seg(buf(w.g_emb), S, S)}};
      SegList gi{1, {seg(buf(w.g_emb0), c.embed_dim, c.embed_dim)}};
      return mlp_bwd(p->blob.embed, c.embed_mlp_depth + 1, go, w.se_h, w.g_se_h, gi, nullptr, 0);
    }
    const SegList none{0, {}};
    ChainArgs ca{};
    ca.nlayers = 3;
    SegList in{2, {seg(buf(w.g_fcat), SL1, S), seg(buf(w.g_w0), W, W)}};
    SegList cn{1, {seg(nullptr, 64, 64)}};
    SegList ad{1, {seg(buf(w.g_aenv), S, S)}};
    SegList zz{1, {seg(buf(w.se_h[0]), 64, 64)}};
    SegList ce{1, {seg(buf(w.g_emb0), c.embed_dim, c.embed_dim)}};
    ca.L[0] = chain_layer(E, in, 0, wt(p->blob.o_g0tq), p->blob.ng0, S, cn, nullptr, nullptr, &ad, 0, 0, 0);
    ca.L[1] = chain_layer(E, none, 0, wt(p->blob.embed.wtq[1]), S, 64, cn, nullptr, &zz, nullptr, 1, 0, 0);
    ca.L[2] = chain_layer(E, none, 0, wt(p->blob.embed.wtq[0]), 64, c.embed_dim, ce, nullptr, nullptr, nullptr, 1, -1, 0);
    auto contract_embedding = [&](ChainLayer& layer, const T* table) {
      layer.embrev_out = buf(w.trev);
      ca.emb_table = table;
      ca.num_types = c.num_types;
      ca.types = g->types;
      ca.center = g->center;
      ca.nbr = g->nbr;
    };
    if (sp.folded_first_stage()) {
      ca.nlayers = 1;
      ca.L[0] = chain_layer(E, in, 0, wt(p->blob.o_g0tfq), p->blob.ng0, 64, cn, nullptr, &zz, &ad, 0, 0, 0);
      if (p->pipe.embed_fused && p->pipe.fold_embed_table) {
        contract_embedding(ca.L[0], wt(p->blob.o_embtab_h));
      } else {
        ca.nlayers = 2;
        ca.L[1] = chain_layer(E, none, 0, wt(p->blob.embed.wtq[0]), 64, c.embed_dim, ce, nullptr, nullptr, nullptr, 1, -1, 0);
      }
    } else if (p->pipe.embed_fused && p->pipe.fold_embed_table) {
      ca.nlayers = 2;
      contract_embedding(ca.L[1], wt(p->blob.o_embtab_h));
    } else if (p->pipe.embed_fused) {
      ca.L[2].g.c = SegList{1, {seg(nullptr, c.embed_dim, c.embed_dim)}};
      contract_embedding(ca.L[2], wt(p->blob.o_embtab));
    }
    return run_chain(ca, "B1");
  }

  int backward(const aa_graph* g, const void* pos, void* forces) {
    if (sp.slot) return backward_slot(g, pos, forces);
    if (int rc = bwd_begin(forces)) return rc;
    if (int rc = bwd_readout(g)) return rc;
    for (int l = p->cfg.num_layers - 1; l >= 0; --l) {
      if (int rc = bwd_latent(l)) return rc;
      if (int rc = bwd_tp_layer(g, l)) return rc;
    }
    if (int rc = bwd_first_stage(g)) return rc;
    return edge_tail(g, pos, forces);
  }
};

struct BlockStep {
  void* vec = nullptr;
  void* dvec = nullptr;
};

template <typename T>
int run_model(const aa_model_plan* p, const void* dev_weights, const aa_graph* g, const void* pos, void* workspace,
              size_t ws_bytes, void* atom_energy, void* forces, hipStream_t stream, StageProfile* prof = nullptr,
              const BlockStep* blk = nullptr) {
  Runner<T> r;
  r.prof = prof;
  if (blk) {
    r.frame_vec = blk->vec;
    r.frame_dvec = blk->dvec;
  }
  r.p = p;
  r.wts = static_cast<const T*>(dev_weights);
  r.ws = static_cast<char*>(workspace);
  r.E = g->num_edges;
  r.N = g->num_atoms;
  r.stream = stream;
  r.e_out = atom_energy;
  r.w = layout_workspace(p, r.N, r.E, forces != nullptr);
  if (r.w.total > ws_bytes) return fail(AA_ERR_WORKSPACE, "aa_model_energy_forces: workspace too small");
  if (p->opt.poison_workspace) AA_CHECK_HIP(hipMemsetAsync(workspace, 0xFF, r.w.total, stream));
  StepInputs in{};
  in.f32 = sizeof(T) == 4;
  in.taps = p->taps;
  in.with_forces = forces != nullptr;
  in.transposed_csr = g->t_rowptr && g->t_perm;
  in.atoms = g->num_atoms;
  in.edges = g->num_edges;
  in.atom0 = r.atom_begin(g);
  in.atom_end = r.atom_end(g);
  in.max_degree = g->max_degree;
  in.pair_zbl = p->zbl_tab != nullptr;
  in.block = blk != nullptr;
  int cus = 0;
  if (wide_one_tile_pass(p->pipe, choose_forward(p->pipe, p->opt, p->cfg, in)) && (cus = device_cu_count()) < 0) return cus;
  r.sp = choose_step(p->pipe, p->opt, p->cfg, in, cus);
  if (p->ev_wait && !blk) AA_CHECK_HIP(hipStreamWaitEvent(stream, (hipEvent_t)(uintptr_t)(p->ev_wait), 0));
  if (int rc = r.forward(g, pos, atom_energy)) return rc;
  if (p->ev_record && !blk) AA_CHECK_HIP(hipEventRecord((hipEvent_t)(uintptr_t)(p->ev_record), stream));
  if (forces) {
    if (int rc = r.backward(g, pos, forces)) return rc;
  } else if (r.sp.pair_zbl) {
    if (int rc = r.pair_zbl(g, pos, nullptr)) return rc;
  }
  if (!blk && g->atom_end > g->atom_begin && (g->atom_begin > 0 || g->atom_end < g->num_atoms) && p->status)
    if (int rc = launch_graph_hint_check(g->rowptr, g->num_atoms, g->atom_begin, g->atom_end, p->status, atom_energy, forces, int(sizeof(T)), stream))
      return rc;
  return AA_OK;
}
}
// ... 282 lines not shown
extern "C" int aa_model_heat_flux(const aa_model_plan* plan, const aa_graph* graph, void* workspace, size_t workspace_bytes,
                                  const void* velocities, void* flux3, aa_stream stream) {
  AA_REQUIRE(plan && graph && workspace, "aa_model_heat_flux: null argument");
  return heat_flux_from(plan, graph, "aa_model_heat_flux", -1, workspace, workspace_bytes, velocities, flux3, stream);
}

extern "C" int aa_model_blocked_heat_flux(const aa_model_plan* plan, const aa_graph* graph, int64_t max_block_edges, void* workspace,
                                          size_t workspace_bytes, const void* velocities, void* flux3, aa_stream stream) {
  AA_REQUIRE(plan && graph && workspace, "aa_model_blocked_heat_flux: null argument");
  AA_REQUIRE(max_block_edges >= 0, "aa_model_blocked_heat_flux: negative max_block_edges");
  return heat_flux_from(plan, graph, "aa_model_blocked_heat_flux", max_block_edges, workspace, workspace_bytes, velocities, flux3, stream);
}

extern "C" int aa_model_frame_energies(const aa_model_plan* plan, const aa_frames* frames, int64_t num_atoms, const void* atom_energy,
                                       void* out_b, aa_stream stream) {
  const char* who = "aa_model_frame_energies";
  AA_REQUIRE(plan, "aa_model_frame_energies: null plan");
  if (int rc = check_frames(frames, who)) return rc;
  AA_REQUIRE(num_atoms >= 0, "aa_model_frame_energies: negative num_atoms");
  AA_REQUIRE(atom_energy || num_atoms == 0, "aa_model_frame_energies: null atom_energy");
  AA_REQUIRE(out_b || frames->num_frames == 0, "aa_model_frame_energies: null output");
  FrameSumArgs a{frames->num_frames, frames->frame_atoms, num_atoms, 0, nullptr, atom_energy, nullptr, nullptr, nullptr, plan->status, out_b};
  return frame_sum(plan, FRAME_ENERGY, a, stream);
}

extern "C" int aa_model_frame_virial(const aa_model_plan* plan, const aa_graph* graph, const aa_frames* frames, void* workspace,
                                     size_t workspace_bytes, void* out_b9, aa_stream stream) {
  AA_REQUIRE(plan && graph && workspace, "aa_model_frame_virial: null argument");
  return frame_edge_sum_from(plan, graph, frames, FRAME_VIRIAL, "aa_model_frame_virial", -1, workspace, workspace_bytes, nullptr, out_b9, stream);
}

extern "C" int aa_model_blocked_frame_virial(const aa_model_plan* plan, const aa_graph* graph, int64_t max_block_edges, const aa_frames* frames,
                                             void* workspace, size_t workspace_bytes, void* out_b9, aa_stream stream) {
  AA_REQUIRE(plan && graph && workspace, "aa_model_blocked_frame_virial: null argument");
  AA_REQUIRE(max_block_edges >= 0, "aa_model_blocked_frame_virial: negative max_block_edges");
  return frame_edge_sum_from(plan, graph, frames, FRAME_VIRIAL, "aa_model_blocked_frame_virial", max_block_edges, workspace, workspace_bytes,
                             nullptr, out_b9, stream);
}

extern "C" int aa_model_frame_heat_flux(const aa_model_plan* plan, const aa_graph* graph, const aa_frames* frames, void* workspace,
                                        size_t workspace_bytes, const void* velocities, void* out_b3, aa_stream stream) {
  AA_REQUIRE(plan && graph && workspace, "aa_model_frame_heat_flux: null argument");
  return frame_edge_sum_from(plan, graph, frames, FRAME_FLUX, "aa_model_frame_heat_flux", -1, workspace, workspace_bytes, velocities, out_b3, stream);
}

extern "C" int aa_model_blocked_frame_heat_flux(const aa_model_plan* plan, const aa_graph* graph, int64_t max_block_edges,
                                                const aa_frames* frames, void* workspace, size_t workspace_bytes, const void* velocities,
                                                void* out_b3, aa_stream stream) {
  AA_REQUIRE(plan && graph && workspace, "aa_model_blocked_frame_heat_flux: null argument");
  AA_REQUIRE(max_block_edges >= 0, "aa_model_blocked_frame_heat_flux: negative max_block_edges");
  return frame_edge_sum_from(plan, graph, frames, FRAME_FLUX, "aa_model_blocked_frame_heat_flux", max_block_edges, workspace, workspace_bytes,
                             velocities, out_b3, stream);
}

extern "C" int aa_model_debug_tap(const aa_model_plan* plan, const char* name, int64_t N, int64_t E, const void* workspace,
                                  const void** ptr, int64_t* ld) {
  AA_REQUIRE(plan && name && workspace && ptr && ld, "aa_model_debug_tap: null argument");
  std::string n(name);
  int with_forces = 0;
  if (n.size() > 2 && n.compare(n.size() - 2, 2, "+f") == 0) {
    with_forces = 1;
    n.resize(n.size() - 2);
  }
  Workspace w = layout_workspace(plan, N, E, with_forces);
  const char* base = static_cast<const char*>(workspace);
  if (n == "edge_attrs") {
    *ptr = base + w.sh;
    *ld = plan->D;
  } else if (n == "edge_embedding") {
    *ptr = base + w.emb;
    *ld = plan->cfg.num_scalar;
  } else if (n == "edge_features") {
    *ptr = base + w.fcat;
    *ld = plan->SL1;
  } else if (n == "emb0") {
    *ptr = base + w.emb0;
    *ld = plan->cfg.embed_dim;
  } else if (n == "vec") {
    *ptr = base + w.vec;
    *ld = 4;
  } else if (n == "dvec" && with_forces) {
    *ptr = base + w.dvec;
    *ld = 4;
  } else {
    return fail(AA_ERR_INVALID, "aa_model_debug_tap: unknown tap");
  }
  return int(*ld);
}
```

### allegro_amd/csrc/aa_tp_spec.hip

```cpp
#include "aa_cg_gen.h"
#include "aa_wave.h"
#include "aa_common.h"

namespace aa {

namespace {

struct LaneMap {
  int64_t atom;
  int ch;
  int width;
  bool valid;
  bool leader;
};

__device__ __forceinline__ LaneMap lane_map(int u, int64_t N) {
  LaneMap m;
  const int tid = threadIdx.x, wave = tid >> 6, lane = tid & 63;
  if (u >= 64) {
    const int wpa = u >> 6;
    m.atom = int64_t(blockIdx.x) * (4 / wpa) + wave / wpa;
    m.ch = (wave % wpa) * 64 + lane;
    m.width = 64;
    m.leader = lane == 0;
// ... 1066 lines not shown
  auto fetch = [&](int s, EdgeIn2<T, D, R>& in) {
    const int sb = s + 1 < end ? s + 1 : s;
    const T* ya = sh + int64_t(s) * a.ld_sh;
    const T* yb = sh + int64_t(sb) * a.ld_sh;
    const T* wa = w0g + int64_t(s) * a.ld_w0;
    const T* wb = w0g + int64_t(sb) * a.ld_w0;
#pragma unroll
    for (int j = 0; j < D; ++j) in.y[j] = T2{ya[j], yb[j]};
#pragma unroll
    for (int r = 0; r < R; ++r) in.wa[r] = T2{ld_stream(wa + r * 64), ld_stream(wb + r * 64)};
  };
  if (beg < end) {
    EdgeIn2<T, D, R> cur, nxt;
    fetch(beg, cur);
    T* sc = static_cast<T*>(a.scal1) + lane;
    for (int s = beg; s < end; s += 2) {
      fetch(s + 2 < end ? s + 2 : s, nxt);
      T2 out[1];
      out[0] = T2{T(0), T(0)};
#pragma unroll
      for (int i = 0; i < Sig0::D1; ++i) out[0] += (cur.y[i] * cur.wa[r_of<0>(i)]) * B1[i];
      st_stream(sc + int64_t(s) * a.ld_scal, out[0][0]);
      if (s + 1 < end) st_stream(sc + int64_t(s + 1) * a.ld_scal, out[0][1]);
      cur = nxt;
    }
  }
}

template <class Sig0, class Sig1, typename T, bool KA2>
__global__ __launch_bounds__(256, (sizeof(T) == 4 && Sig0::LMAX <= 2) ? (KA2 ? 3 : 4) : 1) void tp_mom_bwd_last_kernel(TpMomArgs ma) {
  constexpr int D = Sig0::D2, R = Sig0::LMAX + 1;
  typedef typename Pk<T>::type T2;
  AA_MOM_PROLOGUE(D)
  const T* gs1 = static_cast<const T*>(a.gscal1) + lane;
  T x2s0[D], g2acc[D];
  {
    const T* xi = static_cast<const T*>(a.x2s0) + atom * D * 64 + lane;
#pragma unroll
    for (int j = 0; j < D; ++j) {
      x2s0[j] = xi[int64_t(j) * 64];
      g2acc[j] = T(0);
    }
  }
  T wp0[Sig0::P], wp1[Sig1::P];
  {
    const T* W0 = static_cast<const T*>(a.weights0);
    const T* W1 = static_cast<const T*>(a.weights1);
#pragma unroll
    for (int p = 0; p < Sig0::P; ++p) wp0[p] = a.coupling ? W0[lane * Sig0::P + p] : W0[p];
#pragma unroll
    for (int p = 0; p < Sig1::P; ++p) wp1[p] = a.coupling ? W1[lane * Sig1::P + p] : W1[p];
  }
  T2 Q1[Sig0::D1];
#pragma unroll
  for (int i = 0; i < Sig0::D1; ++i) Q1[i] = T2{T(0), T(0)};
  auto fetch = [&](int s, int ce, PairIn<T, R>& in) {
    const int sa = s < ce ? s : ce - 1, sb = s + 1 < ce ? s + 1 : ce - 1;
    const T* wa = w0g + int64_t(sa) * a.ld_w0;
    const T* wb = w0g + int64_t(sb) * a.ld_w0;
#pragma unroll
    for (int r = 0; r < R; ++r) in.wa[r] = T2{ld_stream(wa + r * 64), ld_stream(wb + r * 64)};
    const T ga = ld_stream(gs1 + int64_t(sa) * a.ld_gscal), gb = ld_stream(gs1 + int64_t(sb) * a.ld_gscal);
    in.g1 = T2{ga, s + 1 < ce ? gb : T(0)};
  };
  mom_pair_loop<T, D, R, 2>(sh, a.ld_sh, beg, end, lane, sY, staged_cb, fetch, [&](int s, bool vb, const T2* y, const PairIn<T, R>& cur) {
#pragma unroll
    for (int i = 0; i < Sig0::D1; ++i) Q1[i] += cur.g1 * (y[i] * cur.wa[r_of<0>(i)]);
  });
  {
    T q[Sig0::D1], tq[Sig0::DOUT], one[1] = {T(1)};
#pragma unroll
    for (int i = 0; i < Sig0::D1; ++i) q[i] = Q1[i][0] + Q1[i][1];
    Sig0::template fwd<T>(q, x2s0, wp0, tq);
    Sig1::template bx2<T>(one, tq, wp1, g2acc);
  }
  const T sf = T(a.sf);
#pragma unroll
  for (int j = 0; j < D; ++j) g2acc[j] *= sf;
  mom_backward_edges<T, D, R, KA2, true>(sh, a.ld_sh, static_cast<const T*>(ma.a1), ma.ld_a1, ma.ka1, true, g2acc,
                              static_cast<const T*>(ma.wt1), beg, end, lane, sM , sY, staged_cb, static_cast<T*>(ma.g_a),
                              ma.ld_ga, static_cast<T*>(a.gsh_env), a.ld_gsh);
}

template <class Sig0, class Sig1, typename T, bool KA2>
#ifndef AA_MOM_FIRST_WAVES
#define AA_MOM_FIRST_WAVES 2
#endif
__global__ __launch_bounds__(256, (sizeof(T) == 4 && Sig0::LMAX <= 2) ? AA_MOM_FIRST_WAVES : 1) void tp_mom_bwd_first_kernel(TpMomArgs ma) {
  constexpr int D = Sig0::D2, D1 = Sig0::D1, DOUT = Sig0::DOUT, R = Sig0::LMAX + 1;
  typedef typename Pk<T>::type T2;
  AA_MOM_PROLOGUE(D)
  const T* gs0 = static_cast<const T*>(a.gscal0);
  const T* gs1 = static_cast<const T*>(a.gscal1);
  const T* w0u = static_cast<const T*>(a.w0);
  const unsigned lane_b0 = unsigned(lane) * unsigned(sizeof(T));
  T x2s0[D], x2s1[D], g2acc[D];
  {
    const int64_t base = atom * D * 64 + lane;
    const T* x0 = static_cast<const T*>(a.x2s0) + base;
    const T* x1p = static_cast<const T*>(a.x2s1) + base;
#pragma unroll
    for (int j = 0; j < D; ++j) {
      x2s0[j] = x0[int64_t(j) * 64];
      x2s1[j] = x1p[int64_t(j) * 64];
      g2acc[j] = T(0);
    }
  }
  T wp0[Sig0::P], wp1[Sig1::P];
  {
    const T* W0 = static_cast<const T*>(a.weights0);
    const T* W1 = static_cast<const T*>(a.weights1);
#pragma unroll
    for (int p = 0; p < Sig0::P; ++p) wp0[p] = a.coupling ? W0[lane * Sig0::P + p] : W0[p];
#pragma unroll
    for (int p = 0; p < Sig1::P; ++p) wp1[p] = a.coupling ? W1[lane * Sig1::P + p] : W1[p];
  }
  T vv[DOUT], B1[D1], B0[D1];
  {
    T one[1] = {T(1)}, e0[DOUT];
#pragma unroll
    for (int k = 0; k < DOUT; ++k) e0[k] = k == 0 ? T(1) : T(0);
    Sig1::template bx1<T>(one, x2s1, wp1, vv);
    Sig0::template bx1<T>(vv, x2s0, wp0, B1);
    Sig0::template bx1<T>(e0, x2s0, wp0, B0);
  }
  T2 Q1[D1], Q0[D1];
#pragma unroll
  for (int i = 0; i < D1; ++i) {
    Q1[i] = T2{T(0), T(0)};
    Q0[i] = T2{T(0), T(0)};
  }
  auto fetch = [&](int s, int ce, PairIn<T, R>& in) {
    const int sa = s < ce ? s : ce - 1, sb = s + 1 < ce ? s + 1 : ce - 1;
    unsigned lane_b = lane_b0;
    opaque_vector(lane_b);
    const T* wa = w0u + int64_t(sa) * a.ld_w0;
    const T* wb = w0u + int64_t(sb) * a.ld_w0;
#pragma unroll
    for (int r = 0; r < R; ++r) in.wa[r] = T2{ld_stream(lane_at(wa + r * 64, lane_b)), ld_stream(lane_at(wb + r * 64, lane_b))};
    const bool vb2 = s + 1 < ce;
    const T g0a = ld_stream(lane_at(gs0 + int64_t(sa) * a.ld_gscal, lane_b)), g0b = ld_stream(lane_at(gs0 + int64_t(sb) * a.ld_gscal, lane_b));
    const T g1a = ld_stream(lane_at(gs1 + int64_t(sa) * a.ld_gscal, lane_b)), g1b = ld_stream(lane_at(gs1 + int64_t(sb) * a.ld_gscal, lane_b));
    in.g0 = T2{g0a, vb2 ? g0b : T(0)};
    in.g1 = T2{g1a, vb2 ? g1b : T(0)};
  };
  T* gw0 = static_cast<T*>(a.g_w0);
  T* gsx = static_cast<T*>(a.gsh_x1);
#ifndef AA_MOM_FIRST_AHEAD
#define AA_MOM_FIRST_AHEAD 1
#endif
  mom_pair_loop<T, D, R, AA_MOM_FIRST_AHEAD>(sh, a.ld_sh, beg, end, lane, sY, staged_cb, fetch, [&](int s, bool vb, const T2* y, const PairIn<T, R>& cur) {
    T2 gw[R];
    T gya[D1], gyb[D1];
#pragma unroll
    for (int r = 0; r < R; ++r) gw[r] = T2{T(0), T(0)};
#pragma unroll
    for (int i = 0; i < D1; ++i) {
      const T2 x1 = y[i] * cur.wa[r_of<0>(i)];
      Q1[i] += cur.g1 * x1;
      Q0[i] += cur.g0 * x1;
      const T2 gx = cur.g1 * B1[i] + cur.g0 * B0[i];
      gw[r_of<0>(i)] += gx * y[i];
      const T2 t = gx * cur.wa[r_of<0>(i)];
      gya[i] = t[0];
      gyb[i] = t[1];
    }
    unsigned lane_b = lane_b0;
    opaque_vector(lane_b);
#pragma unroll
    for (int r = 0; r < R; ++r) st_stream(lane_at(gw0 + int64_t(s) * a.ld_gw0 + r * 64, lane_b), gw[r][0]);
    if (vb) {
#pragma unroll
      for (int r = 0; r < R; ++r) st_stream(lane_at(gw0 + int64_t(s + 1) * a.ld_gw0 + r * 64, lane_b), gw[r][1]);
    }
    wave_sum_store2<T, D1>(gya, gyb, gsx + int64_t(s) * a.ld_gsh, gsx + int64_t(s + (vb ? 1 : 0)) * a.ld_gsh, true, vb);
  });
  {
    T q1[D1], q0[D1], ga[D], gb[D], e0[DOUT];
#pragma unroll
    for (int i = 0; i < D1; ++i) {
      q1[i] = Q1[i][0] + Q1[i][1];
      q0[i] = Q0[i][0] + Q0[i][1];
    }
#pragma unroll
    for (int k = 0; k < DOUT; ++k) e0[k] = k == 0 ? T(1) : T(0);
    Sig0::template bx2<T>(vv, q1, wp0, ga);
    Sig0::template bx2<T>(e0, q0, wp0, gb);
#pragma unroll
    for (int j = 0; j < D; ++j) g2acc[j] = ga[j] + gb[j];
  }
  const T sf = T(a.sf);
#pragma unroll
  for (int j = 0; j < D; ++j) g2acc[j] *= sf;
  mom_backward_edges<T, D, R, KA2, false>(sh, a.ld_sh, static_cast<const T*>(ma.a0), ma.ld_a0, ma.ka0, false, g2acc,
                              static_cast<const T*>(ma.wt0), beg, end, lane, sG, sY, staged_cb, static_cast<T*>(ma.g_a),
                              ma.ld_ga, static_cast<T*>(a.gsh_env), a.ld_gsh);
}

#define AA_FOREACH_CHAIN(X) X(0, Sig1, Sig0) X(1, Sig5, Sig4) X(2, Sig9, Sig8)
int find_chain_pair(int sig0, int sig1) {
  if (sig0 == 1 && sig1 == 0) return 0;
  if (sig0 == 5 && sig1 == 4) return 1;
  if (sig0 == 9 && sig1 == 8) return 2;
  return -1;
}

#define AA_CHAIN_LAUNCHER(NAME)                                                                          \
  template <typename T>                                                                                  \
  int launch_##NAME(int pair, const TpChainArgs& a, hipStream_t stream) {                                \
    if (a.N == 0) return AA_OK;                                                                          \
    dim3 grid(spec_grid(a.u, a.N));                                                                      \
    switch (pair) {                                                                                      \
      case 0: hipLaunchKernelGGL((NAME##_kernel<cg::Sig1, cg::Sig0, T>), grid, dim3(256), 0, stream, a); break; \
      case 1: hipLaunchKernelGGL((NAME##_kernel<cg::Sig5, cg::Sig4, T>), grid, dim3(256), 0, stream, a); break; \
      case 2: hipLaunchKernelGGL((NAME##_kernel<cg::Sig9, cg::Sig8, T>), grid, dim3(256), 0, stream, a); break; \
      default: return fail(AA_ERR_INVALID, #NAME ": unknown chain pair");                                \
    }                                                                                                    \
    AA_CHECK_HIP(hipGetLastError());                                                                     \
    return AA_OK;                                                                                        \
  }                                                                                                      \
  template int launch_##NAME<float>(int, const TpChainArgs&, hipStream_t);                               \
  template int launch_##NAME<double>(int, const TpChainArgs&, hipStream_t);

int find_spec_sig(const aa_tp_desc& d) {
  if (d.mul < 1 || d.mul > 256 || (d.mul & (d.mul - 1)) != 0) return -1;
  for (int sgi = 0; sgi < cg::kNumSigs; ++sgi) {
    const cg::SigInfo& s = cg::kSigs[sgi];
    if (s.d1 != d.d1 || s.d2 != d.d2 || s.dout != d.dout || s.num_paths != d.num_paths || s.nnz != d.nnz) continue;
    bool ok = true;
    for (int n = 0; n < d.nnz && ok; ++n) {
      bool found = false;
      for (int q = 0; q < s.nnz; ++q) {
        if (s.nz[q][0] == d.nz_i[n] && s.nz[q][1] == d.nz_j[n] && s.nz[q][2] == d.nz_k[n] && s.nz[q][3] == d.nz_path[n]) {
          found = std::fabs(s.val[q] - d.nz_val[n]) <= 1e-6 * std::max(1.0, std::fabs(s.val[q]));
          break;
        }
      }
      ok = found;
    }
    if (ok) return sgi;
  }
  return -1;
}


template <typename T>
int launch_tp_spec_fwd(int sig, const TpSpecFwdArgs& a, hipStream_t stream) {
  if (a.N == 0) return AA_OK;
  dim3 grid(spec_grid(a.u, a.N));
  switch (sig) {
#define AA_CASE(ID, SIG)                                                                     \
  case ID:                                                                                   \
    hipLaunchKernelGGL((tp_spec_fwd_kernel<cg::SIG, T>), grid, dim3(256), 0, stream, a);     \
    break;
    AA_FOREACH_SIG(AA_CASE)
#undef AA_CASE
    default:
      return fail(AA_ERR_INVALID, "tp spec fwd: unknown signature");
  }
  AA_CHECK_HIP(hipGetLastError());
  return AA_OK;
}

template <typename T>
int launch_tp_spec_bwd(int sig, const TpSpecBwdArgs& a, hipStream_t stream) {
  if (a.N == 0) return AA_OK;
  dim3 grid(spec_grid(a.u, a.N));
  switch (sig) {
#define AA_CASE(ID, SIG)                                                                     \
  case ID:                                                                                   \
    hipLaunchKernelGGL((tp_spec_bwd_kernel<cg::SIG, T>), grid, dim3(256), 0, stream, a);     \
    break;
    AA_FOREACH_SIG(AA_CASE)
#undef AA_CASE
    default:
      return fail(AA_ERR_INVALID, "tp spec bwd: unknown signature");
  }
  AA_CHECK_HIP(hipGetLastError());
  return AA_OK;
}

#define AA_MOM_LAUNCHER(NAME, K1, K2, K3)                                                                 \
  template <typename T>                                                                                  \
  int launch_##NAME(int pair, const TpMomArgs& a, hipStream_t stream) {                                  \
    if (a.c.N == 0) return AA_OK;                                                                        \
    if (a.c.u != 64 || a.ka0 > kMaxKa || a.ka1 > kMaxKa || (a.ka0 & 63) || (a.ka1 & 63))                \
      return fail(AA_ERR_INVALID, #NAME ": needs u == 64 and env-input widths of 64 or 128");            \
                                                \
    const int wpb = std::max(1, std::min(4, a.waves_per_block));                                                 \
    if (a.c.N <= a.c.atom0) return AA_OK;                                                                \
    dim3 grid((unsigned)((a.c.N - a.c.atom0 + wpb - 1) / wpb));                                          \
    const int dpair = pair == 0 ? 4 : (pair == 1 ? 9 : 16);                                              \
    TpMomArgs b = a;                                                                                     \
    b.ka_lds = a.ka0 > a.ka1 ? a.ka0 : a.ka1;                                                            \
    size_t smem = sizeof(T) * wpb * dpair * (b.ka_lds + 64 + kSegCap);                                   \
    if (smem > 160 * 1024) return fail(AA_ERR_INVALID, #NAME ": LDS patch too large for this dtype/l_max"); \
    if (smem > 64 * 1024) {                                                                              \
      const void* fn = pair == 0 ? (const void*)NAME##_kernel<K1, T, true>                               \
                                 : (pair == 1 ? (const void*)NAME##_kernel<K2, T, true> : (const void*)NAME##_kernel<K3, T, true>); \
      const void* fn1 = pair == 0 ? (const void*)NAME##_kernel<K1, T, false>                             \
                                  : (pair == 1 ? (const void*)NAME##_kernel<K2, T, false> : (const void*)NAME##_kernel<K3, T, false>); \
      AA_CHECK_HIP(hipFuncSetAttribute(fn, hipFuncAttributeMaxDynamicSharedMemorySize, int(smem)));      \
      AA_CHECK_HIP(hipFuncSetAttribute(fn1, hipFuncAttributeMaxDynamicSharedMemorySize, int(smem)));     \
    }                                                                                                    \
    const bool wide = b.ka_lds > 64;                                                                     \
    switch (pair * 2 + (wide ? 1 : 0)) {                                                                 \
      case 0: hipLaunchKernelGGL((NAME##_kernel<K1, T, false>), grid, dim3(64 * wpb), smem, stream, b); break; \
      case 1: hipLaunchKernelGGL((NAME##_kernel<K1, T, true>), grid, dim3(64 * wpb), smem, stream, b); break;  \
      case 2: hipLaunchKernelGGL((NAME##_kernel<K2, T, false>), grid, dim3(64 * wpb), smem, stream, b); break; \
      case 3: hipLaunchKernelGGL((NAME##_kernel<K2, T, true>), grid, dim3(64 * wpb), smem, stream, b); break;  \
      case 4: hipLaunchKernelGGL((NAME##_kernel<K3, T, false>), grid, dim3(64 * wpb), smem, stream, b); break; \
      case 5: hipLaunchKernelGGL((NAME##_kernel<K3, T, true>), grid, dim3(64 * wpb), smem, stream, b); break;  \
      default: return fail(AA_ERR_INVALID, #NAME ": unknown chain pair");                                \
    }                                                                                                    \
    AA_CHECK_HIP(hipGetLastError());                                                                     \
    return AA_OK;                                                                                        \
  }                                                                                                      \
  template int launch_##NAME<float>(int, const TpMomArgs&, hipStream_t);                                 \
  template int launch_##NAME<double>(int, const TpMomArgs&, hipStream_t);
#define AA_COMMA ,
AA_MOM_LAUNCHER(tp_mom_fwd_first, cg::Sig1, cg::Sig5, cg::Sig9)
AA_MOM_LAUNCHER(tp_mom_fwd_last, cg::Sig1 AA_COMMA cg::Sig0, cg::Sig5 AA_COMMA cg::Sig4, cg::Sig9 AA_COMMA cg::Sig8)
AA_MOM_LAUNCHER(tp_mom_bwd_last, cg::Sig1 AA_COMMA cg::Sig0, cg::Sig5 AA_COMMA cg::Sig4, cg::Sig9 AA_COMMA cg::Sig8)
AA_MOM_LAUNCHER(tp_mom_bwd_first, cg::Sig1 AA_COMMA cg::Sig0, cg::Sig5 AA_COMMA cg::Sig4, cg::Sig9 AA_COMMA cg::Sig8)

AA_CHAIN_LAUNCHER(tp_chain_fwd_last)
AA_CHAIN_LAUNCHER(tp_chain_bwd_last)
AA_CHAIN_LAUNCHER(tp_chain_bwd_first)

template int launch_tp_spec_fwd<float>(int, const TpSpecFwdArgs&, hipStream_t);
template int launch_tp_spec_fwd<double>(int, const TpSpecFwdArgs&, hipStream_t);
template int launch_tp_spec_bwd<float>(int, const TpSpecBwdArgs&, hipStream_t);
template int launch_tp_spec_bwd<double>(int, const TpSpecBwdArgs&, hipStream_t);

}
```

### include/allegro_amd.h

```cpp
#ifndef ALLEGRO_AMD_H
#define ALLEGRO_AMD_H

#include <stddef.h>
#include <stdint.h>

#ifdef __cplusplus
extern "C" {
#endif

#if defined(__GNUC__) || defined(__clang__)
#pragma GCC visibility push(default)
#endif

typedef void* aa_stream;

typedef enum { AA_F32 = 0, AA_F64 = 1 } aa_dtype;

enum {
  AA_OK = 0,
  AA_ERR_INVALID = -1,
  AA_ERR_WORKSPACE = -2,
  AA_ERR_HIP = -3
};

// ... 68 lines not shown
  double poly_p;
  int32_t l_max;
  int32_t num_layers;
  int32_t num_scalar;
  int32_t num_tensor;
  int32_t embed_dim;
  int32_t embed_mlp_depth, embed_mlp_width;
  int32_t latent_mlp_depth, latent_mlp_width;
  int32_t readout_mlp_depth, readout_mlp_width;
  int32_t forward_weight_init;
  double avg_num_neighbors;
  double act_const;
  int32_t has_scales, has_shifts;
  aa_tp_desc tps[AA_MAX_LAYERS];
  int32_t embed_kind;
  int32_t spline_span;
  int32_t env_shared_weights;
  int32_t act_kind[3];
  double act_consts[3];
  int32_t bessel_convention;
} aa_model_config;

typedef struct {
  const double* rmax_recip;
  const double* bessel_weights;
  const double* center_embed;
  const double* neighbor_embed;
  const double* basis_linear;
  const double* embed_mlp[AA_MAX_MLP_LAYERS];
  const double* env_embed_linear;
  const double* first_proj;
  const double* latent[AA_MAX_LAYERS][AA_MAX_MLP_LAYERS];
  const double* tp_weights[AA_MAX_LAYERS];
  const double* readout[AA_MAX_MLP_LAYERS];
  const double* scales;
  const double* shifts;
  const double* spline_weights;
} aa_model_raw_weights;

typedef struct {
  int64_t num_atoms;
  int64_t num_edges;
  const int32_t* center;
  const int32_t* nbr;
  const int32_t* rowptr;
  const int32_t* types;
  const void* shift_vec;
  const int32_t* t_rowptr;
  const int32_t* t_perm;
  int64_t atom_begin, atom_end;
  int64_t max_degree;
} aa_graph;

typedef struct aa_model_plan aa_model_plan;

typedef struct {
  int32_t tp_generic;
  int32_t tp_no_chain;
  int32_t tp_no_moments;
  int32_t tp_no_operator;
  int32_t tp_force_operator;
  int32_t tp_operator_fused;
  int32_t gemm_no_chain;
  int32_t gemm_fp32_mfma;
  int32_t gemm_valu;
  int32_t gemm_v1;
  int32_t gemm_lds_epilogue;
  int32_t f64_column_loop;
  int32_t embed_no_fuse;
  int32_t fused_forward;
  int32_t moments_waves_per_block;
  int32_t f64_rows;
  int32_t no_channel_padding;
  int32_t poison_workspace;
  int32_t no_slot_form;
  int32_t op_proj_gemm;
  int32_t op_env_vector;
  int32_t staged_no_fold;
  int32_t op_recompute_bvecs;
  int32_t readout_two_pass;
  int32_t tp_prefer_moments;
  int32_t fused_narrow;
  int32_t chain_staged_weights;
} aa_plan_options;

int aa_model_plan_create(const aa_model_config* cfg, aa_model_plan** out);
int aa_model_plan_create_with_options(const aa_model_config* cfg, const aa_plan_options* options, aa_model_plan** out);
void aa_model_plan_destroy(aa_model_plan* plan);
int aa_model_plan_enable_graph(aa_model_plan* plan, int on);
int aa_model_plan_set_forward_events(aa_model_plan* plan, void* wait_event, void* record_event);
typedef struct {
  int32_t num_types;
  const double* atomic_numbers;
  double qqr2e;
  double poly_p;
} aa_pair_zbl;
int aa_model_plan_set_pair_zbl(aa_model_plan* plan, const aa_pair_zbl* zbl);
int aa_model_plan_enable_taps(aa_model_plan* plan, int on);

size_t aa_model_weights_bytes(const aa_model_plan* plan);
uint64_t aa_model_plan_layout_hash(const aa_model_plan* plan);
int aa_model_pack_weights(const aa_model_plan* plan, const aa_model_raw_weights* raw, void* dev_blob,
                          size_t blob_bytes, aa_stream stream);

size_t aa_model_workspace_bytes(const aa_model_plan* plan, int64_t num_atoms, int64_t num_edges,
                                int with_forces);

int aa_model_energy_forces(const aa_model_plan* plan, const void* dev_weights, const aa_graph* graph,
                           const void* pos, void* workspace, size_t workspace_bytes,
                           void* atom_energy, void* forces, aa_stream stream);

int aa_model_plan_describe(const aa_model_plan* plan, char* buf, size_t buf_bytes);

int aa_model_check(const aa_model_plan* plan, aa_stream stream);

int aa_model_energy_forces_profiled(const aa_model_plan* plan, const void* dev_weights, const aa_graph* graph,
                                    const void* pos, void* workspace, size_t workspace_bytes,
                                    void* atom_energy, void* forces, aa_stream stream, int max_stages,
                                    float* stage_ms, char* stage_names, int* num_stages, double* stage_bytes,
                                    double* stage_flops);

int aa_model_virial(const aa_model_plan* plan, const aa_graph* graph, void* workspace, size_t workspace_bytes,
                    void* virial9, aa_stream stream);

enum { AA_ATOM_VIRIAL_CENTER = 0, AA_ATOM_VIRIAL_NEIGHBOR = 1, AA_ATOM_VIRIAL_SPLIT = 2 };
int aa_model_atom_virial(const aa_model_plan* plan, const aa_graph* graph, void* workspace, size_t workspace_bytes,
                         int attribution, void* out_n9, aa_stream stream);

int aa_model_heat_flux(const aa_model_plan* plan, const aa_graph* graph, void* workspace, size_t workspace_bytes,
                       const void* velocities, void* flux3, aa_stream stream);

size_t aa_model_blocked_workspace_bytes(const aa_model_plan* plan, int64_t num_atoms, int64_t num_edges, int64_t max_block_edges,
                                        int with_forces);
int aa_model_energy_forces_blocked(const aa_model_plan* plan, const void* dev_weights, const aa_graph* graph, const void* pos,
                                   int32_t num_blocks, const int64_t* block_atoms, const int64_t* block_edges, void* workspace,
                                   size_t workspace_bytes, void* atom_energy, void* forces, aa_stream stream);
int aa_model_blocked_virial(const aa_model_plan* plan, const aa_graph* graph, int64_t max_block_edges, void* workspace,
                            size_t workspace_bytes, void* virial9, aa_stream stream);
int aa_model_blocked_atom_virial(const aa_model_plan* plan, const aa_graph* graph, int64_t max_block_edges, void* workspace,
                                 size_t workspace_bytes, int attribution, void* out_n9, aa_stream stream);
int aa_model_blocked_heat_flux(const aa_model_plan* plan, const aa_graph* graph, int64_t max_block_edges, void* workspace,
                               size_t workspace_bytes, const void* velocities, void* flux3, aa_stream stream);

typedef struct aa_frames {
  int32_t num_frames;
  const int32_t* frame_atoms;
} aa_frames;
int aa_model_frame_energies(const aa_model_plan* plan, const aa_frames* frames, int64_t num_atoms, const void* atom_energy, void* out_b,
                            aa_stream stream);
int aa_model_frame_virial(const aa_model_plan* plan, const aa_graph* graph, const aa_frames* frames, void* workspace, size_t workspace_bytes,
                          void* out_b9, aa_stream stream);
int aa_model_frame_heat_flux(const aa_model_plan* plan, const aa_graph* graph, const aa_frames* frames, void* workspace,
                             size_t workspace_bytes, const void* velocities, void* out_b3, aa_stream stream);
int aa_model_blocked_frame_virial(const aa_model_plan* plan, const aa_graph* graph, int64_t max_block_edges, const aa_frames* frames,
                                  void* workspace, size_t workspace_bytes, void* out_b9, aa_stream stream);
int aa_model_blocked_frame_heat_flux(const aa_model_plan* plan, const aa_graph* graph, int64_t max_block_edges, const aa_frames* frames,
                                     void* workspace, size_t workspace_bytes, const void* velocities, void* out_b3, aa_stream stream);

int aa_model_debug_tap(const aa_model_plan* plan, const char* name, int64_t num_atoms, int64_t num_edges,
                       const void* workspace, const void** ptr, int64_t* ld);

typedef struct {
  int64_t num_atoms;
  const void* pos;
  double cell[9];
  int32_t pbc[3];
// ... 156 lines not shown
```

Baseline: 660.8 million edge-TP/s.

## Fuse first-layer moments edge backward into the GEMM chain epilogue

Splits the first-stage moments backward so a per-atom kernel only computes the GM0 per-atom matrix, and moves the per-edge part (dY accumulation and silu-derivative scaling of the latent gradient) into a new epilogue of the bf16x3 chain GEMM. When a 128-row tile spans few centers, the kernel stages their GM0 blocks in LDS. This removes a separate per-edge pass over h, Y and the gradients, at the cost of extra registers and epilogue work in the GEMM. The path turns on by default above an edge-count threshold, and it adds debug taps and an emulator build step.

```diff
diff --git a/__graft_entry__.py b/__graft_entry__.py
--- a/__graft_entry__.py
+++ b/__graft_entry__.py
@@ -16,6 +16,15 @@
 
     lib = ctypes.CDLL(path)
     assert lib.aa_version() >= 1
+    emu_dir = os.path.join(ROOT, "tests", "emu")
+    if os.path.exists(os.path.join(emu_dir, "build_emu.py")):
+        sys.path.insert(0, emu_dir)
+        try:
+            from build_emu import build_emu
+
+            assert os.path.exists(build_emu())
+        finally:
+            sys.path.remove(emu_dir)
     import allegro_amd
     import allegro_amd.nn
     from oracle import restatement
diff --git a/allegro_amd/_lib.py b/allegro_amd/_lib.py
--- a/allegro_amd/_lib.py
+++ b/allegro_amd/_lib.py
@@ -34,7 +34,7 @@
     _fields_ = [(n, C.c_int32) for n in (
         "tp_generic", "tp_no_chain", "tp_no_moments", "tp_no_operator", "tp_force_operator", "tp_operator_fused",
         "gemm_no_chain", "gemm_fp32_mfma", "gemm_valu", "gemm_v1", "gemm_lds_epilogue", "f64_column_loop",
-        "embed_no_fuse", "fused_forward", "moments_waves_per_block", "f64_rows", "no_channel_padding", "poison_workspace", "no_slot_form", "op_proj_gemm", "op_env_vector", "staged_no_fold", "op_recompute_bvecs", "readout_two_pass", "tp_prefer_moments", "fused_narrow", "chain_staged_weights")]
+        "embed_no_fuse", "fused_forward", "moments_waves_per_block", "f64_rows", "no_channel_padding", "poison_workspace", "no_slot_form", "op_proj_gemm", "op_env_vector", "staged_no_fold", "op_recompute_bvecs", "readout_two_pass", "tp_prefer_moments", "fused_narrow", "chain_staged_weights", "mom0_epilogue")]
 
 
 def options_from_env() -> PlanOptions:
@@ -60,6 +60,7 @@
     o.tp_prefer_moments = flag("AA_TP_PREFER_MOM")
     o.fused_narrow = {"1": 1, "2": 2, "3": 3, "4": 4}.get(env.get("AA_FUSED_NARROW", "")[:1], 0)
     o.chain_staged_weights = flag("AA_CHAIN_STAGED")
+    o.mom0_epilogue = {"1": 1, "0": 2}.get(env.get("AA_MOM0_EPILOGUE", "")[:1], 0)
     o.poison_workspace = flag("AA_POISON")
     o.f64_rows = {"0": 2, "2": 1}.get(env.get("AA_F64_ROWS", "")[:1], 0)
     return o
diff --git a/allegro_amd/csrc/aa_common.h b/allegro_amd/csrc/aa_common.h
--- a/allegro_amd/csrc/aa_common.h
+++ b/allegro_amd/csrc/aa_common.h
@@ -235,6 +235,11 @@
   void* edge_sum_out;
   void* kept_out;
   int ld_kept;
+  const void* mom_gm0;
+  const void* mom_y;
+  const void* mom_h;
+  void* mom_dy;
+  int mom_d, ld_mom_y, ld_mom_h, ld_mom_dy;
 };
 struct ChainArgs {
   int64_t M;
@@ -456,6 +461,7 @@
   int ld_ga;
   int ka_lds;
   int waves_per_block;
+  void* gm0;
 };
 struct TpOpArgs {
   int64_t N, E;
@@ -508,6 +514,7 @@
 int launch_tp_mom_bwd_last(int pair, const TpMomArgs& a, hipStream_t stream);
 template <typename T>
 int launch_tp_mom_bwd_first(int pair, const TpMomArgs& a, hipStream_t stream);
+int launch_tp_mom_bwd_first_gm(int pair, const TpMomArgs& a, hipStream_t stream);
 template <typename T>
 int launch_tp_chain_fwd_last(int pair, const TpChainArgs& a, hipStream_t stream);
 template <typename T>
diff --git a/allegro_amd/csrc/aa_gemm.hip b/allegro_amd/csrc/aa_gemm.hip
--- a/allegro_amd/csrc/aa_gemm.hip
+++ b/allegro_amd/csrc/aa_gemm.hip
@@ -1045,6 +1045,9 @@
   int ld_kept, pad3_;
   const float *a2_add, *a2_z;
   int ld_a2add, ld_a2z;
+  const float *mom_gm0, *mom_y, *mom_h;
+  float* mom_dy;
+  int ld_mom_y, ld_mom_h, ld_mom_dy, pad4_;
   const float* a[kChainMaxBlocks];
   int lda[kChainMaxBlocks];
   ChainTileDev t[kChainMaxBlocks];
@@ -1065,8 +1068,10 @@
 };
 
 constexpr int kEpLd = 36;
-
-template <bool PRE, bool EMB>
+constexpr int kChainMomSlots = 8;
+static_assert(kChainMomSlots * 9 * 64 <= 4 * 32 * kEpLd, "the GM0 blocks alias the store-transpose patches");
+
+template <bool PRE, bool EMB, int MOMD = 0>
 __global__ __launch_bounds__(256, PRE ? 2 : 3) void gemm_chain_bf16x3_kernel(ChainDev c) {
   auto chain_split = [](const v4f* a, u32x4* l1, u32x4* l2, u32x4* l3) {
     if constexpr (PRE)
@@ -1097,6 +1102,21 @@
     float* tab = const_cast<float*>(sTab);
     for (int i = tid; i < c.num_types * c.num_types * 512; i += 256) tab[i] = c.emb_table[i];
     sTab += (c.types[c.center[gmc]] * c.num_types + c.types[c.nbr[gmc]]) * 512;
+  }
+  float* sGm = sRo + 32 * kChainMaxBlocks;
+  int mom_c0 = 0;
+  bool mom_lds = false;
+  if constexpr (MOMD > 0) {
+    const ChainLayerDev& ML = c.L[c.nlayers - 1];
+    const int64_t b0 = int64_t(blockIdx.x) * 128, b1 = b0 + 127 < c.M ? b0 + 127 : c.M - 1;
+    mom_c0 = __builtin_amdgcn_readfirstlane(c.center[b0]);
+    const int c1 = __builtin_amdgcn_readfirstlane(c.center[b1]);
+    mom_lds = c1 >= mom_c0 && c1 - mom_c0 < kChainMomSlots;
+    if (mom_lds) {
+      const v4f* src = reinterpret_cast<const v4f*>(ML.mom_gm0 + int64_t(mom_c0) * (MOMD * 64));
+      const int n4 = (c1 - mom_c0 + 1) * (MOMD * 16);
+      for (int i = tid; i < n4; i += 256) reinterpret_cast<v4f*>(sGm)[i] = src[i];
+    }
   }
   auto stage_load = [&](const ChainLayerDev& L, int nt, int kc, u32x4* r) {
     const size_t chunk_stride = 64 * 6, tile_stride = size_t(L.KC) * chunk_stride;
@@ -1239,6 +1259,76 @@
         if (m0 + pr + 8 * q < c.M) *reinterpret_cast<v4f*>(p + int64_t(8 * q) * d.ldc) = v[q];
     }
   };
+  auto mom_epilogue = [&](const ChainLayerDev& L, v16f& acc0, v16f& acc1) {
+    constexpr int D = MOMD > 0 ? MOMD : 1;
+    unsigned ln = unsigned(lane);
+    opaque_vector(ln);
+    const int hh = int(ln >> 5);
+    const int64_t gm = m0 + int64_t(ln & 31u);
+    const bool row_ok = gm < c.M;
+    const int64_t gmc = row_ok ? gm : c.M - 1;
+    v4f za[4], zb[4];
+    {
+      const float* pz = L.mom_h + gmc * L.ld_mom_h + 4 * hh;
+#pragma unroll
+      for (int q = 0; q < 4; ++q) {
+        za[q] = *reinterpret_cast<const v4f*>(pz + 8 * q);
+        zb[q] = *reinterpret_cast<const v4f*>(pz + 32 + 8 * q);
+      }
+    }
+    float Yv[D], gy[D];
+    {
+      const float* py = L.mom_y + gmc * L.ld_mom_y;
+#pragma unroll
+      for (int a = 0; a < D; ++a) {
+        Yv[a] = py[a];
+        gy[a] = 0.f;
+      }
+    }
+    const int ca = c.center[gmc];
+    auto body = [&](const float* bb) {
+#pragma unroll
+      for (int g = 0; g < 8; ++g) {
+        const int q = g & 3;
+        v4f T4 = {0.f, 0.f, 0.f, 0.f}, av;
+#pragma unroll
+        for (int i = 0; i < 4; ++i) av[i] = silu(g < 4 ? za[q][i] : zb[q][i]);
+#pragma unroll
+        for (int a = 0; a < D; ++a) {
+          const v4f b = *reinterpret_cast<const v4f*>(bb + a * 64 + 32 * (g >> 2) + 8 * q);
+#pragma unroll
+          for (int i = 0; i < 4; ++i) {
+            T4[i] += Yv[a] * b[i];
+            gy[a] += av[i] * b[i];
+          }
+        }
+#pragma unroll
+        for (int i = 0; i < 4; ++i) {
+          if (g < 4)
+            acc0[4 * q + i] = (acc0[4 * q + i] + T4[i]) * dsilu(za[q][i]);
+          else
+            acc1[4 * q + i] = (acc1[4 * q + i] + T4[i]) * dsilu(zb[q][i]);
+        }
+        if (g < 4)
+          anchor(acc0);
+        else
+          anchor(acc1);
+#pragma unroll
+        for (int a = 0; a < D; ++a) anchor(gy[a]);
+        __builtin_amdgcn_sched_barrier(0);
+      }
+    };
+    const float* gmb = L.mom_gm0 + int64_t(ca) * (D * 64);
+    if (mom_lds) gmb = sGm + (ca - mom_c0) * (D * 64);
+    body(gmb + 4 * hh);
+#pragma unroll
+    for (int a = 0; a < D; ++a) gy[a] += __shfl_xor(gy[a], 32);
+    if (row_ok && hh == 0) {
+      float* gb = L.mom_dy + gm * L.ld_mom_dy;
+#pragma unroll
+      for (int a = 0; a < D; ++a) gb[a] = gy[a];
+    }
+  };
 
   const float* const dummy_a = c.L[0].a[0];
   const int dummy_lda = c.L[0].lda[0];
@@ -1303,7 +1393,7 @@
                    (lastc && !kernel_end) ? 0 : (kernel_end ? kc : kc + 1), r);
         u32x4 x1[2], x2[2], x3[2];
         if (!pre) {
-          if (kc >= KCg) {
+          if (MOMD == 0 && kc >= KCg) {
             v4f a[4];
             kept_a(L, kc - KCg, a);
             chain_split(a, x1, x2, x3);
@@ -1347,8 +1437,13 @@
 #endif
         ++step;
       }
-      epilogue(L.t[nt], acc0);
-      if (two) epilogue(L.t[nt + 1], acc1);
+      if constexpr (MOMD > 0) {
+        if (L.mom_gm0) mom_epilogue(L, acc0, acc1);
+      }
+      if constexpr (MOMD == 0) {
+        epilogue(L.t[nt], acc0);
+        if (two) epilogue(L.t[nt + 1], acc1);
+      }
       if (EMB && L.embrev_out) {
         float part[8];
 #pragma unroll
@@ -1368,12 +1463,19 @@
         for (int n = 0; n < 8; ++n) other[n] = part[n];
         permlane32_swap4(part, other);
         permlane32_swap4(part + 4, other + 4);
+        int64_t gms = gm;
+        if constexpr (MOMD > 0) {
+          unsigned l2 = unsigned(lane);
+          opaque_vector(l2);
+          gms = m0 + int64_t(l2 & 31u);
+        }
         if (row_ok) {
           const int o4 = 4 * hh;
-          *reinterpret_cast<v4f*>(L.embrev_out + gm * 8 + o4) =
+          *reinterpret_cast<v4f*>(L.embrev_out + gms * 8 + o4) =
               v4f{part[o4] + other[o4], part[o4 + 1] + other[o4 + 1], part[o4 + 2] + other[o4 + 2], part[o4 + 3] + other[o4 + 3]};
         }
       }
+      if constexpr (MOMD > 0) return;
       if (L.edge_sum_out) {
         float part = 0.f;
 #pragma unroll
@@ -1387,7 +1489,7 @@
         permlane32_swap(t, o);
         if (row_ok && hh == 0) L.edge_sum_out[gm] = t + o;
       }
-      if (nt == L.keep_tile) {
+      if (MOMD == 0 && nt == L.keep_tile) {
 #pragma unroll
         for (int r = 0; r < 16; ++r) {
           kept0[r] = L.keep_act ? silu(acc0[r]) : acc0[r];
@@ -1423,6 +1525,7 @@
     return fail(AA_ERR_INVALID, "gemm chain: the embedding table needs 1..2 types and the edge / type arrays");
   if (c.nlayers < 1 || c.nlayers > 4) return fail(AA_ERR_INVALID, "gemm chain: 1..4 layers");
   bool have_kept = false;
+  int mom_d = 0;
   static_assert(sizeof(ChainDev) <= 4096, "kernel argument block too large");
   for (int li = 0; li < c.nlayers; ++li) {
     const ChainLayer& L = c.L[li];
@@ -1497,6 +1600,20 @@
       return fail(AA_ERR_INVALID, "gemm chain: kept_out needs a kept tile pair and 16-B aligned rows");
     D.embrev_out = static_cast<float*>(L.embrev_out);
     if (L.embrev_out && (!c.emb_table || g.N != 64)) return fail(AA_ERR_INVALID, "gemm chain: embrev_out needs the table and a 64-wide layer");
+    if (L.mom_gm0) {
+      auto al16 = [](const void* q) { return (reinterpret_cast<uintptr_t>(q) & 15) == 0; };
+      if (c.nlayers != 1 || L.use_prev || L.kept_out || g.N != 64 || g.has_z || g.has_add || (L.mom_d != 4 && L.mom_d != 9) || !L.mom_y || !L.mom_h || !L.mom_dy ||
+          !c.center || !al16(L.mom_gm0) || !al16(L.mom_h) || (L.ld_mom_h & 3) || L.ld_mom_y < L.mom_d || L.ld_mom_dy < L.mom_d)
+        return fail(AA_ERR_INVALID, "gemm chain: the moments epilogue needs a chain of one 64-wide layer without z / add operands, D = 4 or 9 and its arrays");
+      D.mom_gm0 = static_cast<const float*>(L.mom_gm0);
+      D.mom_y = static_cast<const float*>(L.mom_y);
+      D.mom_h = static_cast<const float*>(L.mom_h);
+      D.mom_dy = static_cast<float*>(L.mom_dy);
+      D.ld_mom_y = L.ld_mom_y;
+      D.ld_mom_h = L.ld_mom_h;
+      D.ld_mom_dy = L.ld_mom_dy;
+      mom_d = L.mom_d;
+    }
     D.edge_sum_out = static_cast<float*>(L.edge_sum_out);
     if (L.edge_sum_out) {
       if (!c.ro_w || g.N != 64) return fail(AA_ERR_INVALID, "gemm chain: edge_sum_out needs ro_w and a 64-wide layer");
@@ -1511,7 +1628,16 @@
   bool emb = false;
   for (int li = 0; li < d.nlayers; ++li) emb = emb || d.L[li].embrev_out != nullptr;
 #define AA_CHAIN_LAUNCH(P_, E_) hipLaunchKernelGGL((gemm_chain_bf16x3_kernel<P_, E_>), grid, dim3(256), smem, stream, d)
-  if (any_pre) {
+  if (mom_d) {
+    bool stores = false;
+    for (int li = 0; li < d.nlayers; ++li)
+      for (int t = 0; t < d.L[li].NT; ++t) stores = stores || d.L[li].t[t].c != nullptr;
+    if (stores || any_pre || !emb) return fail(AA_ERR_INVALID, "gemm chain: the moments epilogue needs a chain that stores no tile and contracts the embedding");
+    if (mom_d == 4)
+      hipLaunchKernelGGL((gemm_chain_bf16x3_kernel<false, true, 4>), grid, dim3(256), smem, stream, d);
+    else
+      hipLaunchKernelGGL((gemm_chain_bf16x3_kernel<false, true, 9>), grid, dim3(256), smem, stream, d);
+  } else if (any_pre) {
     if (emb) AA_CHAIN_LAUNCH(true, true); else AA_CHAIN_LAUNCH(true, false);
   } else {
     if (emb) AA_CHAIN_LAUNCH(false, true); else AA_CHAIN_LAUNCH(false, false);
diff --git a/allegro_amd/csrc/aa_model.hip b/allegro_amd/csrc/aa_model.hip
--- a/allegro_amd/csrc/aa_model.hip
+++ b/allegro_amd/csrc/aa_model.hip
@@ -336,6 +336,7 @@
   bool gather;
   bool zero_gsh, zero_forces;
   bool pair_zbl;
+  bool mom0_in_chain;
   bool block;
 
   bool fused() const { return forward == ForwardKind::FusedOneTile || forward == ForwardKind::FusedTeam || forward == ForwardKind::FusedMixed; }
@@ -372,6 +373,7 @@
   return pipe.fused_wide && (forward == ForwardKind::FusedOneTile || forward == ForwardKind::FusedMixed);
 }
 
+constexpr int64_t kMom0EpilogueEdges = int64_t(256) * 3 * 128;
 static StepPlan choose_step(const ModelPipeline& pipe, const aa_plan_options& opt, const aa_model_config& c, const StepInputs& in, int cus) {
   const int64_t n = in.atom_end - in.atom0;
   const bool two_layer_chains = pipe.chains() && c.num_layers == 2;
@@ -397,6 +399,10 @@
                      : !(pipe.fold_lat0_reverse && c.num_layers == 2)                ? LatentReverse::TwoLayerChain
                      : (resident_shape && !opt.chain_staged_weights)                 ? LatentReverse::Resident
                                                                                      : LatentReverse::FoldedChain;
+
+  const bool mom0_ok = in.with_forces && in.f32 && s.folded_first_stage() && pipe.tp == TpPath::Moments && pipe.chains() && pipe.embed_fused &&
+                       pipe.fold_embed_table && (pipe.chain_pair == 0 || pipe.chain_pair == 1) && c.num_scalar == 64;
+  s.mom0_in_chain = mom0_ok && opt.mom0_epilogue != 2 && (opt.mom0_epilogue == 1 || in.edges >= kMom0EpilogueEdges);
 
   s.op_split = pipe.tp_op >= 0 && !opt.tp_operator_fused;
   s.op_split_reverse = s.op_split && in.with_forces;
@@ -1336,7 +1342,9 @@
     for (int i = 0; i < c.latent_mlp_depth; ++i) w.g_lat_h[i] = take(Ez * c.latent_mlp_width);
     for (int l = 0; l < L; ++l) w.g_scal[l] = take(Ez * u);
     if (!p->pipe.env_moments()) w.g_envw = take(Ez * p->W);
-    if (p->pipe.env_moments()) w.g_aenv = take(Ez * size_t(std::max(S, c.latent_mlp_width)));
+    const bool gm0_here = p->pipe.tp == TpPath::Moments && p->pipe.chains() && p->pipe.embed_fused && p->pipe.fold_embed_table && es == 4;
+    if (p->pipe.env_moments())
+      w.g_aenv = take(std::max(Ez * size_t(std::max(S, c.latent_mlp_width)), gm0_here ? Nz * p->D * 64 : size_t(0)));
     w.g_w0 = take(Ez * p->W);
     if (L > 1 && p->pipe.chain_pair < 0) {
       w.g_tf[0] = take(Ez * u * dmax);
@@ -1653,15 +1661,20 @@
     if (!prof) return AA_OK;
     char nm[32];
     int o = snprintf(nm, sizeof(nm), "gc");
-    double elems = 0, fl = 0;
+    double elems = 0, fl = 0, per_atom = 0;
     for (int i = 0; i < ca.nlayers; ++i) {
       if (o < 28) o += snprintf(nm + o, sizeof(nm) - o, "_%dx%d", ca.L[i].g.K, ca.L[i].g.N);
       elems += gemm_row_elems(ca.L[i].g, true);
       if (ca.L[i].a_mode == 2) elems += 2.0 * ca.L[i].g.a.s[0].n;
       fl += 2.0 * double(E) * ca.L[i].g.K * ca.L[i].g.N;
+      if (ca.L[i].mom_gm0) {
+        elems += 64 + 2.0 * ca.L[i].mom_d;
+        per_atom += 64.0 * ca.L[i].mom_d;
+        fl += 4.0 * double(E) * ca.L[i].mom_d * 64;
+      }
     }
     (void)tag;
-    return mark(nm, elems, 0, fl);
+    return mark(nm, elems, per_atom, fl);
   }
 
   TpMomArgs mom_args(const aa_graph* g) const {
@@ -2434,6 +2447,11 @@
         }
         m.ld_ga = S;
         if (sp.folded_first_stage()) m.wt0 = wt(p->blob.o_wt0f);
+        if (sp.mom0_in_chain) {
+          m.gm0 = buf(w.g_aenv);
+          if (int rc = launch_tp_mom_bwd_first_gm(p->pipe.chain_pair, m, stream)) return rc;
+          return mark("tp_mom_bwd_first", p->D + 2 * W + 2 * u + p->D, double(p->D) * 64, 2.0 * p->D * u);
+        }
         if (int rc = launch_tp_mom_bwd_first<T>(p->pipe.chain_pair, m, stream)) return rc;
         return mark("tp_mom_bwd_first", p->D + 2 * W + 2 * u + 2 * m.ka0 + 2 * p->D, 2.0 * p->D * u);
       }
@@ -2537,6 +2555,17 @@
     if (sp.folded_first_stage()) {
       ca.nlayers = 1;
       ca.L[0] = chain_layer(E, in, 0, wt(p->blob.o_g0tfq), p->blob.ng0, 64, cn, nullptr, &zz, &ad, 0, 0, 0);
+      if (sp.mom0_in_chain) {
+        ca.L[0] = chain_layer(E, in, 0, wt(p->blob.o_g0tfq), p->blob.ng0, 64, cn, nullptr, nullptr, nullptr, 0, 0, 0);
+        ca.L[0].mom_gm0 = buf(w.g_aenv);
+        ca.L[0].mom_d = p->D;
+        ca.L[0].mom_y = buf(w.sh);
+        ca.L[0].ld_mom_y = p->D;
+        ca.L[0].mom_h = buf(w.se_h[0]);
+        ca.L[0].ld_mom_h = 64;
+        ca.L[0].mom_dy = buf(w.g_sh) + size_t(E) * p->D;
+        ca.L[0].ld_mom_dy = p->D;
+      }
       if (p->pipe.embed_fused && p->pipe.fold_embed_table) {
         contract_embedding(ca.L[0], wt(p->blob.o_embtab_h));
       } else {
@@ -2985,6 +3014,12 @@
   } else if (n == "dvec" && with_forces) {
     *ptr = base + w.dvec;
     *ld = 4;
+  } else if (n == "gsh_env0" && with_forces && plan->pipe.channel_minor() && plan->pipe.tp_op < 0 && plan->cfg.num_layers >= 1) {
+    *ptr = base + w.g_sh + size_t(E) * plan->D * plan->esize();
+    *ld = plan->D;
+  } else if (n == "trev" && with_forces && plan->pipe.embed_fused) {
+    *ptr = base + w.trev;
+    *ld = 8;
   } else {
     return fail(AA_ERR_INVALID, "aa_model_debug_tap: unknown tap");
   }
diff --git a/allegro_amd/csrc/aa_tp_spec.hip b/allegro_amd/csrc/aa_tp_spec.hip
--- a/allegro_amd/csrc/aa_tp_spec.hip
+++ b/allegro_amd/csrc/aa_tp_spec.hip
@@ -1172,7 +1172,7 @@
                               ma.ld_ga, static_cast<T*>(a.gsh_env), a.ld_gsh);
 }
 
-template <class Sig0, class Sig1, typename T, bool KA2>
+template <class Sig0, class Sig1, typename T, bool KA2, bool GM_ONLY = false>
 #ifndef AA_MOM_FIRST_WAVES
 #define AA_MOM_FIRST_WAVES 2
 #endif
@@ -1282,6 +1282,18 @@
   const T sf = T(a.sf);
 #pragma unroll
   for (int j = 0; j < D; ++j) g2acc[j] *= sf;
+  if constexpr (GM_ONLY) {
+    __builtin_amdgcn_wave_barrier();
+#pragma unroll
+    for (int j = 0; j < D; ++j) sG[j * 64 + lane] = g2acc[j];
+    __builtin_amdgcn_wave_barrier();
+    T gm[D];
+    mom_gm_plain<T, D, R>(sG, static_cast<const T*>(ma.wt0), ma.ka0, 0, lane, gm);
+    T* out = static_cast<T*>(ma.gm0) + atom * D * 64 + lane;
+#pragma unroll
+    for (int j = 0; j < D; ++j) out[int64_t(j) * 64] = gm[j];
+    return;
+  }
   mom_backward_edges<T, D, R, KA2, false>(sh, a.ld_sh, static_cast<const T*>(ma.a0), ma.ld_a0, ma.ka0, false, g2acc,
                               static_cast<const T*>(ma.wt0), beg, end, lane, sG, sY, staged_cb, static_cast<T*>(ma.g_a),
                               ma.ld_ga, static_cast<T*>(a.gsh_env), a.ld_gsh);
@@ -1414,6 +1426,24 @@
 AA_MOM_LAUNCHER(tp_mom_bwd_last, cg::Sig1 AA_COMMA cg::Sig0, cg::Sig5 AA_COMMA cg::Sig4, cg::Sig9 AA_COMMA cg::Sig8)
 AA_MOM_LAUNCHER(tp_mom_bwd_first, cg::Sig1 AA_COMMA cg::Sig0, cg::Sig5 AA_COMMA cg::Sig4, cg::Sig9 AA_COMMA cg::Sig8)
 
+int launch_tp_mom_bwd_first_gm(int pair, const TpMomArgs& a, hipStream_t stream) {
+  if (a.c.N == 0 || a.c.N <= a.c.atom0) return AA_OK;
+  if (a.c.u != 64 || a.ka0 != 64 || a.ka1 != 64 || !a.gm0 || (pair != 0 && pair != 1))
+    return fail(AA_ERR_INVALID, "tp_mom_bwd_first_gm: needs u == 64, env-input widths of 64, l_max <= 2 and the GM0 array");
+  const int wpb = std::max(1, std::min(4, a.waves_per_block));
+  dim3 grid((unsigned)((a.c.N - a.c.atom0 + wpb - 1) / wpb));
+  const int dpair = pair == 0 ? 4 : 9;
+  TpMomArgs b = a;
+  b.ka_lds = 64;
+  const size_t smem = sizeof(float) * wpb * dpair * (b.ka_lds + 64 + kSegCap);
+  if (pair == 0)
+    hipLaunchKernelGGL((tp_mom_bwd_first_kernel<cg::Sig1, cg::Sig0, float, false, true>), grid, dim3(64 * wpb), smem, stream, b);
+  else
+    hipLaunchKernelGGL((tp_mom_bwd_first_kernel<cg::Sig5, cg::Sig4, float, false, true>), grid, dim3(64 * wpb), smem, stream, b);
+  AA_CHECK_HIP(hipGetLastError());
+  return AA_OK;
+}
+
 AA_CHAIN_LAUNCHER(tp_chain_fwd_last)
 AA_CHAIN_LAUNCHER(tp_chain_bwd_last)
 AA_CHAIN_LAUNCHER(tp_chain_bwd_first)
diff --git a/include/allegro_amd.h b/include/allegro_amd.h
--- a/include/allegro_amd.h
+++ b/include/allegro_amd.h
@@ -174,6 +174,7 @@
   int32_t tp_prefer_moments;
   int32_t fused_narrow;
   int32_t chain_staged_weights;
+  int32_t mom0_epilogue;
 } aa_plan_options;
 
 int aa_model_plan_create(const aa_model_config* cfg, aa_model_plan** out);
```

Result: faster. 683.9 million edge-TP/s, median of 6 (+3.5%).
